# proycon/analiticcl

Hardware: AMD Instinct MI355X
Metric: scored (query,candidate) pairs/sec + queries/sec, 200k-lexicon, len≤16, 1/2/4/8 GPU (higher is better)
Workload: dtype u8

## Files before the change

analiticcl_amd/_lib.py:

```python
from __future__ import annotations

import ctypes as C
import os

HERE = os.path.dirname(os.path.abspath(__file__))
LIB_PATH = os.environ.get("ANX_LIB") or os.path.join(HERE, "libanx.so")

ANX_OK, ANX_EINVAL, ANX_EIO, ANX_ENOTBUILT, ANX_ENODEVICE, ANX_ELIMIT, ANX_EEMPTY = 0, -1, -2, -3, -4, -5, -6
ANX_NO_VIA = 0xFFFFFFFFFFFFFFFF
ABI_VERSION = 3


class AnxError(RuntimeError):
    def __init__(self, code: int, message: str):
        super().__init__(f"anx error {code}: {message}")
        self.code = code


class Weights(C.Structure):
    _fields_ = [("ld", C.c_double), ("lcs", C.c_double), ("prefix", C.c_double), ("suffix", C.c_double),
                ("casew", C.c_double)]


class Threshold(C.Structure):
# ... 92 lines not shown
        "anx_index_read_tag": (C.c_void_p, [cp]),
        "anx_model_num_lexicons": (u64, [vp]),
        "anx_model_lexicon_name": (cp, [vp, u64]),
        "anx_model_to_device": (C.c_int, [vp, C.c_int]),
        "anx_model_to_devices": (C.c_int, [vp, C.POINTER(C.c_int), C.c_int]),
        "anx_model_num_replicas": (C.c_int, [vp]),
        "anx_model_replica_device": (C.c_int, [vp, C.c_int]),
        "anx_debug_set_switch": (C.c_int, [cp, cp]),
        "anx_batch_num_shards": (C.c_int, [vp]),
        "anx_batch_shard_info": (C.c_int, [vp, C.c_int, C.POINTER(C.c_int), C.POINTER(sz), C.POINTER(sz)]),
        "anx_batch_shard_inputs": (C.c_int, [vp, C.c_int, C.POINTER(C.POINTER(C.c_uint32))]),
        "anx_model_has": (C.c_int, [vp, cp]),
        "anx_model_vocab_size": (u64, [vp]),
        "anx_model_vocab_text": (cp, [vp, u64]),
        "anx_model_vocab_frequency": (C.c_uint32, [vp, u64]),
        "anx_model_vocab_lexindex": (C.c_uint32, [vp, u64]),
        "anx_model_num_instances": (u64, [vp]),
        "anx_model_num_classes": (u64, [vp]),
        "anx_model_bucket_size": (u64, [vp, C.c_int]),
        "anx_model_alphabet_size": (C.c_int, [vp]),
        "anx_model_normalize": (C.c_int, [vp, cp, C.c_char_p, C.c_int]),
        "anx_model_anahash": (C.c_int, [vp, cp, C.c_char_p, C.c_int]),
        "anx_find_variants_batch": (C.c_int, [vp, C.POINTER(cp), sz, C.POINTER(Params),
                                              C.POINTER(C.POINTER(Result)), C.POINTER(C.POINTER(sz))]),
        "anx_results_free": (None, [C.POINTER(Result), C.POINTER(sz)]),
        "anx_format_query_output": (C.c_int, [vp, C.POINTER(cp), sz, C.POINTER(Result), C.POINTER(sz), C.c_float, C.c_int,
                                              C.c_int, u64, C.POINTER(C.c_void_p), C.POINTER(sz)]),
        "anx_string_free": (None, [C.c_void_p]),
        "anx_format_search_output": (C.c_int, [vp, C.POINTER(cp), sz, C.POINTER(Match), C.POINTER(sz), C.POINTER(Result),
                                               C.POINTER(MatchTag), C.c_float, C.c_int, C.c_int, u64,
                                               C.POINTER(C.c_void_p), C.POINTER(sz)]),
        "anx_default_search_params": (None, [C.POINTER(SearchParams)]),
        "anx_find_all_matches_batch": (C.c_int, [vp, C.POINTER(cp), sz, C.POINTER(SearchParams),
                                                 C.POINTER(C.POINTER(Match)), C.POINTER(C.POINTER(sz)),
                                                 C.POINTER(C.POINTER(Result)), C.POINTER(sz),
                                                 C.POINTER(C.POINTER(MatchTag))]),
        "anx_matches_free": (None, [C.POINTER(Match), C.POINTER(sz), C.POINTER(Result), C.POINTER(MatchTag)]),
        "anx_model_add_contextrule": (C.c_int, [vp, cp, C.c_float, C.POINTER(cp), sz, C.POINTER(cp), sz]),
        "anx_model_read_contextrules": (C.c_int, [vp, cp]),
        "anx_model_num_tags": (sz, [vp]),
        "anx_model_tag_name": (cp, [vp, sz]),
        "anx_batch_encode": (vp, [vp, C.POINTER(cp), sz, C.POINTER(Params)]),
        "anx_batch_encode_packed": (vp, [vp, C.c_char_p, sz, sz, C.POINTER(Params)]),
        "anx_batch_gather_compact": (C.c_int, [vp, C.c_int, vp, sz, C.POINTER(sz), C.POINTER(sz)]),
        "anx_batch_encode_packed_device": (vp, [vp, vp, sz, sz, C.POINTER(Params)]),
        "anx_batch_encode_packed_device_on": (vp, [vp, vp, sz, sz, C.POINTER(Params), vp]),
        "anx_debug_search_stats": (C.c_int, [C.POINTER(C.c_uint64)]),
        "anx_learn_variants": (C.c_int, [vp, C.POINTER(cp), sz, C.POINTER(Params), C.c_int, C.POINTER(C.c_uint64)]),
        "anx_learn_variants_search": (C.c_int, [vp, C.POINTER(cp), sz, C.POINTER(SearchParams), C.c_int, C.POINTER(C.c_uint64)]),
        "anx_learn_apply_rows": (C.c_int, [vp, C.POINTER(cp), sz, C.POINTER(Result), C.POINTER(sz), C.POINTER(C.c_uint64)]),
        "anx_model_variants": (C.c_int64, [vp, u64, C.POINTER(C.c_uint8), C.POINTER(C.c_uint64), C.POINTER(C.c_double), sz]),
        "anx_model_vocab_type": (C.c_uint32, [vp, u64]),
        "anx_format_variant_list": (C.c_int, [vp, C.c_int, C.POINTER(C.c_void_p)]),
        "anx_debug_learn_stats": (C.c_int, [C.POINTER(C.c_uint64)]),
        "anx_debug_learn_times": (C.c_int, [C.POINTER(C.c_double)]),
        "anx_debug_small_stats": (C.c_int, [C.POINTER(C.c_uint64)]),
        "anx_batch_run": (C.c_int, [vp, vp, vp]),
        "anx_batch_run_async": (C.c_int, [vp, vp, vp]),
        "anx_batch_wait": (C.c_int, [vp, vp]),
        "anx_batch_fetch": (C.c_int, [vp, C.POINTER(C.POINTER(Result)), C.POINTER(C.POINTER(sz))]),
        "anx_batch_fetch_compact": (C.c_int, [vp, C.POINTER(C.c_void_p), C.POINTER(C.POINTER(C.c_uint32))]),
        "anx_compact_free": (None, [C.c_void_p, C.POINTER(C.c_uint32)]),
        "anx_compact_to_results": (None, [C.c_void_p, sz, C.POINTER(Result)]),
        "anx_batch_fetch_pairs": (C.c_int, [vp, C.POINTER(C.POINTER(Pair)), C.POINTER(sz)]),
        "anx_pairs_free": (None, [C.POINTER(Pair)]),
        "anx_batch_pair_counts": (C.c_int, [vp, C.POINTER(C.POINTER(C.c_uint32))]),
        "anx_counts_free": (None, [C.POINTER(C.c_uint32)]),
        "anx_batch_export_topk": (C.c_int, [vp, vp, C.c_uint32, vp]),
        "anx_batch_export_compact": (C.c_int, [vp, vp, sz, vp, C.POINTER(sz)]),
        "anx_batch_get_stats": (C.c_int, [vp, C.POINTER(BatchStats), C.c_size_t]),
        "anx_shutdown": (None, []),
        "anx_pipeline_new": (vp, [vp, C.c_int]),
        "anx_pipeline_submit_packed": (C.c_int, [vp, cp, C.c_size_t, C.c_size_t, C.POINTER(Params)]),
        "anx_pipeline_pending": (C.c_int, [vp]),
        "anx_pipeline_next": (C.c_int, [vp, C.POINTER(vp), C.POINTER(C.POINTER(C.c_uint32)), C.POINTER(C.c_size_t)]),
        "anx_pipeline_free": (None, [vp]),
        "anx_debug_kernel_timer": (None, [C.c_int]),
        "anx_debug_kernel_time": (C.c_int, [cp, C.POINTER(C.c_double), C.POINTER(C.c_uint64)]),
        "anx_debug_length_split": (C.c_int, [vp, C.POINTER(C.c_char_p), C.c_size_t, C.POINTER(Params), C.c_int, vp, vp]),
        "anx_debug_signature": (C.c_int, [vp, cp, C.POINTER(C.c_uint64)]),
        "anx_debug_entries": (C.c_int, [vp, C.POINTER(C.POINTER(C.c_uint32)), C.POINTER(C.c_size_t)]),
        "anx_debug_adjacency": (C.c_int, [vp, C.c_int, C.c_uint64, vp, C.c_size_t, vp, C.POINTER(C.POINTER(C.c_uint32)), vp]),
        "anx_debug_adjacency_device": (C.c_int, [vp, vp, C.c_size_t, vp, C.POINTER(C.POINTER(C.c_uint32))]),
        "anx_debug_band_bound": (C.c_int, [C.c_int, vp, vp, vp, vp, C.c_size_t, C.c_int, C.c_int, vp]),
        "anx_batch_free": (None, [vp]),
        "anx_device_pool_trim": (None, [C.c_int]),
    }
    for name, (res, args) in sig.items():
        fn = getattr(L, name)
        fn.restype = res
        fn.argtypes = args
    _lib = L
    return L


EXPORTED = None


def set_switch(name: str, value) -> None:
    check(lib().anx_debug_set_switch(name.encode(), None if value is None else str(value).encode()))


def kernel_timer(enable: bool) -> None:
    lib().anx_debug_kernel_timer(1 if enable else 0)


def kernel_time(name: str):
    ms, n = C.c_double(0.0), C.c_uint64(0)
    lib().anx_debug_kernel_time(name.encode(), C.byref(ms), C.byref(n))
    return ms.value, n.value


def check(rc: int):
    if rc != 0:
        raise AnxError(rc, lib().anx_last_error().decode("utf-8", "replace"))


def last_error() -> str:
    return lib().anx_last_error().decode("utf-8", "replace")
```

analiticcl_amd/csrc/adjacency.h:

```cpp
#pragma once
#include <cstdint>
#include <cstddef>
#include <vector>

namespace anx {

struct LexiconImage;

constexpr int kAdjRadius = 3;
constexpr int kAdjSections = 2 * kAdjRadius + 1;
constexpr int kAdjMaxClosure = 2;
constexpr uint32_t kAdjRow = 64;

struct AdjHdr {
  uint32_t row0;
  uint32_t cum[kAdjSections];
};
struct AdjSlot {
  uint32_t lo, hi;
  uint32_t hdr1;
  uint32_t rows;
};
struct AdjPlanes { uint32_t p1, p2; };

struct AdjIndex {
  std::vector<AdjSlot> hash;
  uint32_t hash_mask = 0;
  std::vector<AdjHdr> hdr;
  AdjPlanes* planes = nullptr;
  uint32_t* ids = nullptr;
  uint64_t rows = 0;
  uint32_t nsig_lexicon = 0, nsig_closure = 0, nsig_kept = 0;
  uint64_t records = 0;
  uint64_t rows_wanted = 0;
  double len_records[256] = {};
  std::vector<float> class_records;
  std::vector<float> class_nsig;
  double build_ms = 0.0;
  AdjIndex() = default;
  AdjIndex(const AdjIndex&) = delete;
  AdjIndex& operator=(const AdjIndex&) = delete;
  ~AdjIndex();
  uint32_t find(uint32_t lo, uint32_t hi) const;
};

void build_adjacency(const LexiconImage& img, int closure, size_t budget_bytes, unsigned threads, AdjIndex& out);

}
```

analiticcl_amd/csrc/capi.cpp:

```cpp
#include <chrono>
#include <cmath>
#include <cstdlib>
#include <charconv>
#include <cstring>
#include <fstream>
#include <sstream>
#include <string>

#include "engine.h"
#include <algorithm>
#include <atomic>
#include <condition_variable>
#include <deque>
#include <functional>
#include <memory>
#include <mutex>
#include <thread>

#include "host_model.h"

namespace {
struct Worker {
  std::thread th;
  std::mutex mu;
// ... 292 lines not shown
    adj.reset(new anx::AdjIndex());
    anx::build_adjacency(m->host.lex, anx::switches().adj_closure, (size_t)anx::switches().adj_budget_mb << 20, anx::usable_hw_threads(), *adj);
  }
  auto publish = [&](const anx::AdjIndex& a, bool have) {
    LengthCost& lc = m->len_cost;
    std::lock_guard<std::mutex> lk(lc.mu);
    for (uint32_t L = 0; L < LengthCost::LMAX; ++L) lc.records[L] = a.len_records[L];
    lc.class_records = a.class_records;
    lc.class_nsig = a.class_nsig;
    lc.have_records = have;
    lc.init = false;
    if (getenv("ANX_ADJ_TIMING"))
      fprintf(stderr, "[anx adjacency] %s: %u lexicon signatures, %u in the closure, %u lists, %llu records in %llu rows (%.1f MB), %.1f ms\n", on_device ? "device" : "host",
              a.nsig_lexicon, a.nsig_closure, a.nsig_kept, (unsigned long long)a.records, (unsigned long long)a.rows, a.rows * 64.0 * 12.0 / 1e6, a.build_ms);
  };
  if (adj) publish(*adj, !adj->hash.empty());
  for (int i = 0; i < n; ++i) {
    Replica r;
    r.device = devices[i];
    if (on_device && i == 0) stats.reset(new anx::AdjIndex());
    r.dev = anx::lexicon_upload(m->host.lex, et, adj.get(), devices[i], err, on_device ? anx::switches().adj_closure : -1, (size_t)anx::switches().adj_budget_mb << 20,
                                (on_device && i == 0) ? stats.get() : nullptr);
    if (r.dev && on_device && i == 0) publish(*stats, stats->nsig_kept != 0);
    if (r.dev && n > 1 && !(r.stream = anx::stream_create(devices[i], err))) { anx::lexicon_free(r.dev); r.dev = nullptr; }
    if (!r.dev) { drop_replicas(m); return fail(ANX_ENODEVICE, err); }
    if (n > 1) r.worker.reset(new Worker());
    m->replicas.push_back(std::move(r));
  }
  m->dev = m->replicas[0].dev;
  return ANX_OK;
}
int anx_model_to_device(anx_model* m, int device) { return anx_model_to_devices(m, &device, 1); }
int anx_model_num_replicas(const anx_model* m) { return m ? (int)m->replicas.size() : 0; }
int anx_model_replica_device(const anx_model* m, int i) { return (m && i >= 0 && (size_t)i < m->replicas.size()) ? m->replicas[(size_t)i].device : -1; }
int anx_debug_signature(const anx_model* m, const char* utf8, uint64_t* out_sig) {
  if (!m || !utf8 || !out_sig) return fail(ANX_EINVAL, "NULL argument");
  if (!m->host.built) return fail(ANX_ENOTBUILT, "Model has not been built yet!");
  std::vector<uint8_t> norm, cv;
  if (!m->host.encode(utf8, norm, cv)) return fail(ANX_ELIMIT, "more than 255 symbols");
  cv.resize((size_t)m->host.lex.nplanes * 4, 0);
  *out_sig = anx::signature_of(cv.data(), cv.size(), m->host.lex.sym_group);
  return ANX_OK;
}
int anx_debug_entries(const anx_model* m, uint32_t** out_vocab_ids, size_t* n) {
  if (!m || !out_vocab_ids || !n) return fail(ANX_EINVAL, "NULL argument");
  if (!m->host.built) return fail(ANX_ENOTBUILT, "Model has not been built yet!");
  const std::vector<uint32_t>& v = m->host.lex.ent_vocab;
  uint32_t* o = static_cast<uint32_t*>(malloc(std::max<size_t>(v.size(), 1) * sizeof(uint32_t)));
  if (!o) return fail(ANX_ELIMIT, "out of memory");
  if (!v.empty()) memcpy(o, v.data(), v.size() * sizeof(uint32_t));
  *out_vocab_ids = o;
  *n = v.size();
  return ANX_OK;
}
int anx_debug_adjacency(const anx_model* m, int closure, uint64_t budget_bytes, const uint64_t* sigs, size_t n, uint32_t* out_cum, uint32_t** out_ids,
                        uint64_t* out_stats) {
  if (!m || (!sigs && n) || (!out_cum && n) || !out_ids) return fail(ANX_EINVAL, "NULL argument");
  if (!m->host.built) return fail(ANX_ENOTBUILT, "Model has not been built yet!");
  anx::AdjIndex adj;
  anx::build_adjacency(m->host.lex, closure, (size_t)budget_bytes, anx::usable_hw_threads(), adj);
  if (out_stats) { out_stats[0] = adj.nsig_lexicon; out_stats[1] = adj.nsig_closure; out_stats[2] = adj.nsig_kept; out_stats[3] = adj.records; out_stats[4] = adj.rows; out_stats[5] = (uint64_t)adj.build_ms; out_stats[6] = adj.rows_wanted; }
  size_t total = 0;
  std::vector<uint32_t> h1(n);
  for (size_t i = 0; i < n; ++i) {
    h1[i] = adj.find((uint32_t)sigs[i], (uint32_t)(sigs[i] >> 32));
    if (h1[i]) total += (size_t)adj.hdr[h1[i] - 1].cum[anx::kAdjSections - 1] * anx::kAdjRow;
  }
  uint32_t* ids = static_cast<uint32_t*>(malloc(std::max<size_t>(total, 1) * sizeof(uint32_t)));
  if (!ids) return fail(ANX_ELIMIT, "out of memory");
  size_t pos = 0;
  for (size_t i = 0; i < n; ++i) {
    uint32_t* c = out_cum + i * (anx::kAdjSections + 1);
    if (!h1[i]) { for (int s = 0; s <= anx::kAdjSections; ++s) c[s] = 0xFFFFFFFFu; continue; }
    const anx::AdjHdr& h = adj.hdr[h1[i] - 1];
    c[0] = (uint32_t)(pos / anx::kAdjRow);
    for (int s = 0; s < anx::kAdjSections; ++s) c[s + 1] = h.cum[s];
    const size_t cnt = (size_t)h.cum[anx::kAdjSections - 1] * anx::kAdjRow;
    memcpy(ids + pos, adj.ids + (size_t)h.row0 * anx::kAdjRow, cnt * sizeof(uint32_t));
    pos += cnt;
  }
  *out_ids = ids;
  return ANX_OK;
}
int anx_debug_adjacency_device(const anx_model* m, const uint64_t* sigs, size_t n, uint32_t* out_cum, uint32_t** out_ids) {
  if (!m || (!sigs && n) || (!out_cum && n) || !out_ids) return fail(ANX_EINVAL, "NULL argument");
  if (m->replicas.empty()) return fail(ANX_ENODEVICE, "model is not resident on a device");
  std::string err;
  const int rc = anx::adjacency_debug_lists(m->replicas[0].dev, sigs, n, out_cum, out_ids, err);
  return rc ? fail(rc, err) : ANX_OK;
}
int anx_debug_set_switch(const char* name, const char* value) {
  return anx::set_switch(name, value) ? ANX_OK : fail(ANX_EINVAL, "unknown switch");
}
void anx_debug_kernel_timer(int enable) { anx::kernel_timer_enable(enable != 0); }
int anx_debug_small_stats(uint64_t* out) { if (!out) return fail(ANX_EINVAL, "NULL argument"); anx::small_stats(out); return ANX_OK; }
int anx_debug_kernel_time(const char* name, double* total_ms, uint64_t* launches) {
  return anx::kernel_timer_read(name, total_ms, launches) ? ANX_OK : fail(ANX_EINVAL, "no launch of that kernel was timed");
}
int anx_debug_band_bound(int device, const uint8_t* q_rows, const uint8_t* c_rows, const uint8_t* lq, const uint8_t* lc, size_t n, int d, int form,
                         uint8_t* out_reject) {
  if ((!q_rows || !c_rows || !lq || !lc || !out_reject) && n) return fail(ANX_EINVAL, "NULL argument");
  std::string err;
  const int rc = anx::debug_band_bound(device, q_rows, c_rows, lq, lc, n, d, form, out_reject, err);
  return rc ? fail(rc, err) : ANX_OK;
}
int anx_model_build(anx_model* m, int device) {
  if (!m) return fail(ANX_EINVAL, "NULL model");
  std::string err;
  int rc = m->host.build_index(err);
  if (rc) return fail(rc, err);
  drop_replicas(m);
  if (device < 0) return ANX_OK;
  return anx_model_to_device(m, device);
}
int anx_model_save_index(const anx_model* m, const char* path) {
  if (!m || !path) return fail(ANX_EINVAL, "NULL argument");
  std::string err;
  const int rc = m->host.save_index(path, err);
  return rc ? fail(rc, err) : ANX_OK;
}
int anx_model_set_index_tag(anx_model* m, const char* tag) {
  if (!m || !tag) return fail(ANX_EINVAL, "NULL argument");
  m->host.index_tag = tag;
  return ANX_OK;
}
char* anx_index_read_tag(const char* path) {
  if (!path) { fail(ANX_EINVAL, "NULL argument"); return nullptr; }
  std::string tag, err;
  const int rc = anx::index_read_tag(path, &tag, err);
  if (rc) { fail(rc, err); return nullptr; }
  char* out = static_cast<char*>(malloc(tag.size() + 1));
  if (!out) { fail(ANX_EINVAL, "out of memory"); return nullptr; }
  memcpy(out, tag.c_str(), tag.size() + 1);
  return out;
}
int anx_model_load_index(anx_model* m, const char* path, int device) {
  if (!m || !path) return fail(ANX_EINVAL, "NULL argument");
  std::string err;
  const int rc = m->host.load_index(path, err);
  if (rc) return fail(rc, err);
  drop_replicas(m);
  if (device < 0) return ANX_OK;
  return anx_model_to_device(m, device);
}
uint64_t anx_model_num_lexicons(const anx_model* m) { return m ? m->host.lexicons.size() : 0; }
const char* anx_model_lexicon_name(const anx_model* m, uint64_t i) {
  return (m && i < m->host.lexicons.size()) ? m->host.lexicons[i].c_str() : nullptr;
}
int anx_model_has(const anx_model* m, const char* utf8) { return (m && utf8 && m->host.has(utf8)) ? 1 : 0; }
uint64_t anx_model_vocab_size(const anx_model* m) { return m ? m->host.decoder.size() : 0; }
const char* anx_model_vocab_text(const anx_model* m, uint64_t id) {
  return (m && id < m->host.decoder.size()) ? m->host.decoder[id].text.c_str() : nullptr;
}
uint32_t anx_model_vocab_frequency(const anx_model* m, uint64_t id) {
  return (m && id < m->host.decoder.size()) ? m->host.decoder[id].frequency : 0;
}
uint32_t anx_model_vocab_lexindex(const anx_model* m, uint64_t id) {
  return (m && id < m->host.decoder.size()) ? m->host.decoder[id].lexindex : 0;
}
uint64_t anx_model_num_instances(const anx_model* m) { return m ? m->host.lex.nentries : 0; }
uint64_t anx_model_num_classes(const anx_model* m) { return m ? m->host.lex.nclasses : 0; }
uint64_t anx_model_bucket_size(const anx_model* m, int c) {
  if (!m || !m->host.built || c < 0 || c > anx::kMaxSymbols) return 0;
  return m->host.lex.bucket_begin[c + 1] - m->host.lex.bucket_begin[c];
}
int anx_model_alphabet_size(const anx_model* m) { return m ? m->host.alphabet_size() : 0; }
// ... 1404 lines not shown
```

analiticcl_amd/csrc/encode.hip:

```cpp
#include <hip/hip_runtime.h>

#include <cstdio>
#include <cstring>
#include <ctime>
#include <string>
#include <vector>

#include <rocprim/device/device_radix_sort.hpp>
#include <rocprim/device/device_scan.hpp>

#include "engine_internal.h"

namespace anx {

#define HIP_TRY(expr)                                                                          \
  do {                                                                                         \
    hipError_t _e = (expr);                                                                    \
    if (_e != hipSuccess) {                                                                    \
      err = std::string(#expr) + ": " + hipGetErrorString(_e);                                 \
      return ANX_ENODEVICE;                                                                    \
    }                                                                                          \
  } while (0)

#include "kernels_common.hpp"
// ... 295 lines not shown
  const uint32_t meta = g.meta[i], len = meta & 0xFFu;
  const unsigned long long sig = g.sig[i];
  g.q_meta[s] = meta;
  g.q_orig[s] = i;
  g.s_sig[s] = sig;
  static_assert(NBITPLANES == 4, "planes move as one uint4");
  const uint4 planes = reinterpret_cast<const uint4*>(g.bits)[i];
  const uint32_t kind = g.kind[i];
  reinterpret_cast<uint4*>(g.q_bits)[s] = planes;
  g.s_kind[s] = kind;
  if (kind == 0)
    for (int p = 0; p < g.NP; ++p) g.q_cv[(size_t)s * g.NP + p] = g.cv[(size_t)i * g.NP + p];
  const uint32_t* __restrict__ src = reinterpret_cast<const uint32_t*>(g.codes + code_off(g.off[i], i));
  for (uint32_t w = 0; w < g.qw; ++w) {
    const uint32_t left = len > w * 16u ? len - w * 16u : 0u;
    uint32_t v[4];
#pragma unroll
    for (uint32_t x = 0; x < 4u; ++x) {
      const uint32_t word = 4u * x < left ? src[w * 4u + x] : 0u;
      const uint32_t valid = left > 4u * x ? left - 4u * x : 0u;
      const uint32_t mask = valid >= 4u ? 0xFFFFFFFFu : (1u << (8u * valid)) - 1u;
      v[x] = (word & mask) | (0xFEFEFEFEu & ~mask);
    }
    const uint4 row = make_uint4(v[0], v[1], v[2], v[3]);
    g.q_rows[(size_t)s * g.qw + w] = row;
    if (w == 0) {
      uint32_t pw[3] = {0u, 0u, 0u};
      {
        uint32_t p[6] = {0u, 0u, 0u, 0u, 0u, 0u};
#pragma unroll
        for (uint32_t i = 0; i < 16u; ++i) {
          const uint32_t c = ((v[i >> 2] >> (8u * (i & 3u))) & 0xFFu) + 1u;
          const uint32_t on = i < len ? 1u : 0u;
#pragma unroll
          for (uint32_t b = 0; b < 6u; ++b) p[b] |= (((c >> b) & on)) << i;
        }
        pw[0] = p[0] | p[1] << 16; pw[1] = p[2] | p[3] << 16; pw[2] = p[4] | p[5] << 16;
      }
      g.q_rec[2 * (size_t)s] = row;
      g.q_rec[2 * (size_t)s + 1] = make_uint4(meta, pw[0], pw[1], pw[2]);
    }
  }
  uint32_t xc = 0xFFFFFFFFu;
  if (g.want_exact) {
    int lo = (int)g.siglen_begin[len], hi = (int)g.siglen_begin[len + 1] - 1;
    while (lo <= hi) {
      const int mid = (lo + hi) >> 1;
      const uint4 r = g.sigtab[mid];
      const unsigned long long v = (unsigned long long)r.x | (unsigned long long)r.y << 32;
      if (sig < v) hi = mid - 1;
      else if (sig > v) lo = mid + 1;
      else {
        for (uint32_t c = r.z; c < r.z + r.w && xc == 0xFFFFFFFFu; ++c) {
          bool eq = true;
          for (int p = 0; p < g.NP; ++p)
            eq = eq && g.cls_planes[(size_t)p * g.cstride + c] == (kind ? cv_word_of_planes(planes, (uint32_t)p) : g.cv[(size_t)i * g.NP + p]);
          if (eq) xc = c;
        }
        break;
      }
    }
  }
  g.qexact[s] = xc;
}
__global__ __launch_bounds__(256) void k_enc_gather(GatherArgs g) {
  const uint32_t s = blockIdx.x * 256 + threadIdx.x;
  if (s < g.nq) enc_gather_body(g, s);
}

struct TileArgs {
  uint32_t nq, tq;
  const uint32_t *q_meta, *s_kind;
  const unsigned long long* s_sig;
  const uint32_t* siglen_begin;
  uint32_t* head;
  uint32_t* tcount;
  Tile* tiles;
  uint32_t* tkey;
  uint32_t* ctr;
  const uint32_t* ball_tab;
  int probe;
  const uint4* adj_hash;
  uint32_t adj_mask;
};
__device__ inline uint32_t adj_lookup(const uint4* tab, uint32_t mask, uint32_t lo, uint32_t hi, uint32_t* rows) {
  if (!mask) return 0u;
  uint32_t h = sig_hash(lo, hi) & mask;
  for (int p = 0; p < 17; ++p) {
    const uint4 e = tab[h];
    if (!e.z) return 0u;
    if (e.x == lo && e.y == hi) { *rows = e.w; return e.z; }
    h = (h + 1u) & mask;
  }
  return 0u;
}
__device__ inline bool same_segment(const TileArgs& t, uint32_t a, uint32_t b) {
  return (t.s_kind[a] == 0) == (t.s_kind[b] == 0) && (t.q_meta[a] & 0xFFu) == (t.q_meta[b] & 0xFFu) && t.s_sig[a] == t.s_sig[b];
}
__device__ inline void tile_window(const TileArgs& t, uint32_t s, uint32_t& s0, uint32_t& s1, uint32_t& step, uint32_t& nparts,
                                   uint32_t& ball0, uint32_t& balln) {
  const uint32_t meta = t.q_meta[s], lq = meta & 0xFFu, k = (meta >> 8) & 0xFFu;
  const int lo = max(1, (int)lq - (int)k), hi = min(kMaxSymbols, (int)lq + (int)k);
  s0 = t.siglen_begin[lo] & ~63u;
  s1 = (t.siglen_begin[hi + 1] + 63u) & ~63u;
  ball0 = balln = 0;
  if (t.probe && k <= 12u && tile_probes(t.ball_tab[13 + k], s1 - s0, t.s_sig[s])) { ball0 = t.ball_tab[k]; balln = t.ball_tab[13 + k]; }
  const uint32_t nsplit = (t.s_kind[s] == 0 && !balln) ? 8u : 1u;
  step = (((s1 - s0) + nsplit - 1u) / nsplit + 63u) & ~63u;
  nparts = 0;
  for (uint32_t part = 0; part < nsplit; ++part) {
    const uint32_t a0 = s0 + part * step, a1 = min(s1, a0 + step);
    if (a0 >= a1 && part) break;
    ++nparts;
  }
}
__global__ __launch_bounds__(256) void k_tile_heads(TileArgs t) {
  const uint32_t s = blockIdx.x * 256 + threadIdx.x;
  if (s >= t.nq) return;
  t.head[s] = (s > 0 && !same_segment(t, s, s - 1)) ? s : 0u;
}
__global__ __launch_bounds__(256) void k_tile_count(TileArgs t) {
  const uint32_t s = blockIdx.x * 256 + threadIdx.x;
  if (s > t.nq) return;
  uint32_t c = 0;
  if (s < t.nq && (s - t.head[s]) % t.tq == 0) {
    uint32_t s0, s1, step, nparts, ball0, balln;
    tile_window(t, s, s0, s1, step, nparts, ball0, balln);
    c = nparts;
  }
  t.tcount[s] = c;
}
__global__ __launch_bounds__(256) void k_tile_emit(TileArgs t) {
  const uint32_t s = blockIdx.x * 256 + threadIdx.x;
  if (s >= t.nq || (s - t.head[s]) % t.tq != 0) return;
  const uint32_t hs = t.head[s];
  uint32_t lo = s + 1u, hi = min(s + t.tq, t.nq);
  while (lo < hi) {
    const uint32_t mid = (lo + hi) >> 1;
    if (t.head[mid] != hs) hi = mid; else lo = mid + 1u;
  }
  const uint32_t tn = lo - s;
  uint32_t ke[3];
#pragma unroll
  for (uint32_t v = 1; v <= 3u; ++v) {
    uint32_t a = s, b = s + tn;
    while (a < b) {
      const uint32_t mid = (a + b) >> 1;
      if (t.s_kind[mid] > v) b = mid; else a = mid + 1u;
    }
    ke[v - 1] = a - s;
  }
  const bool sad = t.s_kind[s] == 0;
  const uint32_t meta = t.q_meta[s], lq = meta & 0xFFu, k = (meta >> 8) & 0xFFu, d = (meta >> 16) & 0xFFu;
  uint32_t s0, s1, step, nparts, ball0, balln;
  tile_window(t, s, s0, s1, step, nparts, ball0, balln);
  const unsigned long long sig = t.s_sig[s];
  const uint32_t base = t.tcount[s];
  uint32_t adj_rows = 0;
  const uint32_t adj = (!sad && k <= (uint32_t)kAdjRadius) ? adj_lookup(t.adj_hash, t.adj_mask, (uint32_t)sig, (uint32_t)(sig >> 32), &adj_rows) : 0u;
  for (uint32_t part = 0; part < nparts; ++part) {
    const uint32_t a0 = s0 + part * step, a1 = min(s1, a0 + step);
    Tile tl;
    tl.q0 = s; tl.nq = tn; tl.s0 = a0; tl.s1 = a1; tl.k = k; tl.lq = lq; tl.sig_lo = (uint32_t)sig; tl.sig_hi = (uint32_t)(sig >> 32);
    tl.kind = sad ? 0u : 1u; tl.d = d; tl.kend = sad ? 0u : (ke[0] | ke[1] << 8 | ke[2] << 16);
    tl.ball0 = ball0; tl.balln = balln; tl.adj = adj; tl.flags = (s == hs && part == 0u) ? 1u : 0u;
    t.tiles[base + part] = tl;
    const unsigned long long cost = adj ? (unsigned long long)adj_rows * (8u + tn) + 16u : (unsigned long long)tn * (a1 - a0 + 64u);
    t.tkey[base + part] = (sad ? 0x80000000u : adj ? 0u : 0x40000000u) | (0x3FFFFFFFu - (uint32_t)(cost < 0x3FFFFFFFull ? cost : 0x3FFFFFFFull));
  }
  if (sad) atomicAdd(&t.ctr[3], nparts);
}

__global__ __launch_bounds__(256) void k_tile_adj_count(const Tile* tiles, uint32_t n, uint32_t* ctr) {
  const uint32_t i = blockIdx.x * 256 + threadIdx.x;
  if (i < n && tiles[i].adj && (i + 1 == n || !tiles[i + 1].adj)) ctr[5] = i + 1u;
}

__global__ __launch_bounds__(256) void k_small_tiles(GatherArgs g, TileArgs t, SmallZero z, uint32_t slots, const uint32_t* __restrict__ adj_hdr) {
  const uint32_t s = blockIdx.x * 256 + threadIdx.x, nthreads = gridDim.x * 256u;
#pragma unroll
  for (int a = 0; a < 8; ++a)
    for (uint32_t i = s; i < z.n[a]; i += nthreads) z.p[a][i] = 0u;
  if (s >= t.nq) return;
  enc_gather_body(g, s);
  const uint32_t meta = t.q_meta[s], lq = meta & 0xFFu, k = (meta >> 8) & 0xFFu, d = (meta >> 16) & 0xFFu;
  Tile nul{};
  nul.kind = 1u;
  uint32_t nparts = 0;
  if (meta) {
    const uint32_t kind = t.s_kind[s];
    const bool sad = kind == 0;
    uint32_t s0, s1, step, ball0, balln;
    tile_window(t, s, s0, s1, step, nparts, ball0, balln);
    const unsigned long long sig = t.s_sig[s];
    uint32_t adj_rows = 0;
    const uint32_t adj = (!sad && k <= (uint32_t)kAdjRadius) ? adj_lookup(t.adj_hash, t.adj_mask, (uint32_t)sig, (uint32_t)(sig >> 32), &adj_rows) : 0u;
    uint32_t rbeg = 0, rend = 0;
    if (adj) {
      const uint32_t* hp = adj_hdr + (size_t)(adj - 1u) * 8u;
      rbeg = k >= 3u ? 0u : k == 2u ? hp[1] : k == 1u ? hp[2] : hp[3];
      rend = k >= 3u ? hp[7] : k == 2u ? hp[6] : k == 1u ? hp[5] : hp[4];
      const uint32_t rows = rend > rbeg ? rend - rbeg : 0u;
      nparts = min(slots, max(1u, rows / 8u));
      step = ((rows + nparts - 1u) / nparts + 3u) & ~3u;
    }
    for (uint32_t part = 0; part < nparts; ++part) {
      const uint32_t a0 = s0 + part * step, a1 = min(s1, a0 + step);
      Tile tl;
      tl.q0 = s; tl.nq = 1u; tl.s0 = a0; tl.s1 = a1; tl.k = k; tl.lq = lq; tl.sig_lo = (uint32_t)sig; tl.sig_hi = (uint32_t)(sig >> 32);
      tl.kind = sad ? 0u : 1u; tl.d = d;
      tl.kend = sad ? 0u : ((kind <= 1u ? 1u : 0u) | (kind <= 2u ? 1u : 0u) << 8 | (kind <= 3u ? 1u : 0u) << 16);
      tl.ball0 = ball0; tl.balln = balln; tl.adj = adj; tl.flags = part == 0u ? 1u : 0u;
      if (adj) {
        tl.s0 = min(rend, rbeg + part * step);
        tl.s1 = min(rend, tl.s0 + step);
        tl.flags |= 2u;
        if (tl.s0 >= tl.s1 && part) tl.nq = 0u;
      }
      t.tiles[(size_t)part * t.nq + s] = tl;
    }
  }
  (void)nul;
  for (uint32_t part = nparts; part < slots; ++part) t.tiles[(size_t)part * t.nq + s].nq = 0u;
}

int small_encode_launch(const HostModel& m, const DeviceLexicon* dl, const SmallEnc& e, const uint8_t* blob, const uint32_t* off, uint32_t n, uint32_t qw,
                        const anx_params& p, const SmallZero& z, uint32_t slots, bool stage_lds, const uint32_t* host_off, hipStream_t st, std::string& err) {
  const int NP = dl->nplanes;
  EncArgs ea;
  ea.blob = blob; ea.off = off; ea.n = n; ea.al = dl->alpha; ea.A = m.alphabet.size(); ea.NP = NP;
  ea.bits_ok = (dl->nsym <= 32 && !switches().scan_sad) ? 1 : 0;
  ea.ngroups = 1;
  for (uint8_t g : m.lex.sym_group) ea.ngroups = std::max(ea.ngroups, (int)g + 1);
  ea.kth = p.max_anagram_distance; ea.dth = p.max_edit_distance;
  ea.codes = e.codes; ea.meta = e.meta; ea.bits = e.bits; ea.sig = e.sig; ea.kind = e.kind; ea.cv = e.cv; ea.key = e.key; ea.blk = e.blk;
  ea.dbg = 0;
  ea.zero_cv = 1;
  for (uint32_t bk = 0; bk <= 16u; ++bk) ea.stage_off[bk] = host_off ? host_off[std::min<uint32_t>(bk * 256u, n)] : 0u;
  const dim3 gn((n + 255) / 256);
  if (stage_lds && host_off && n <= 4096u) hipLaunchKernelGGL(k_enc_strings<true>, gn, dim3(256), 0, st, ea);
  else hipLaunchKernelGGL(k_enc_strings<false>, gn, dim3(256), 0, st, ea);
  GatherArgs ga;
  ga.nq = n; ga.qw = qw; ga.NP = NP; ga.want_exact = 0;
  ga.perm = e.perm; ga.off = off; ga.codes = e.codes; ga.meta = e.meta; ga.bits = e.bits; ga.kind = e.kind; ga.cv = e.cv; ga.sig = e.sig;
  ga.q_rec = e.q_rec; ga.q_rows = e.q_rows; ga.q_bits = e.q_bits; ga.q_cv = e.q_cv; ga.q_meta = e.q_meta; ga.q_orig = e.q_orig;
  ga.qexact = e.qexact; ga.s_kind = e.s_kind; ga.s_sig = e.s_sig;
  ga.sigtab = dl->sig; ga.siglen_begin = dl->alpha.siglen_begin; ga.cls_planes = dl->cls_planes; ga.cstride = dl->cstride;
  TileArgs ta;
  ta.tq = 1; ta.nq = n; ta.q_meta = e.q_meta; ta.s_kind = e.s_kind; ta.s_sig = e.s_sig; ta.siglen_begin = dl->alpha.siglen_begin; ta.ctr = nullptr;
  ta.ball_tab = dl->ball_tab; ta.probe = probe_enabled() ? 1 : 0;
  ta.adj_hash = dl->adj_hash; ta.adj_mask = switches().scan_adj ? dl->adj_mask : 0u;
  ta.head = nullptr; ta.tcount = nullptr; ta.tiles = e.tiles; ta.tkey = nullptr;
  hipLaunchKernelGGL(k_small_tiles, gn, dim3(256), 0, st, ga, ta, z, slots, dl->adj_hdr);
  HIP_TRY(hipGetLastError());
  return ANX_OK;
}
int small_iota(uint32_t* perm, uint32_t n, hipStream_t st) {
  hipLaunchKernelGGL(k_iota, dim3((n + 255) / 256), dim3(256), 0, st, perm, n);
  return hipGetLastError() == hipSuccess ? ANX_OK : ANX_ENODEVICE;
}

namespace {
struct Scratch {
  std::vector<void*> blocks;
  int device;
  hipStream_t st;
  explicit Scratch(int dev) : device(dev), st(encoder_stream_acquire(dev)) {}
  template <typename T>
  int get(T** p, size_t count, std::string& err) {
    void* q = nullptr;
    HIP_TRY(pool_malloc(&q, std::max<size_t>(count * sizeof(T), 16)));
    blocks.push_back(q);
    *p = static_cast<T*>(q);
    return ANX_OK;
  }
  ~Scratch() { (void)hipStreamSynchronize(st); for (void* q : blocks) pool_free(q); encoder_stream_release(device, st); }
};
template <typename K>
int sort_pairs(const K* kin, K* kout, const uint32_t* vin, uint32_t* vout, size_t n, unsigned b0, unsigned b1, Scratch& sc, hipStream_t st,
               std::string& err) {
  size_t bytes = 0;
  HIP_TRY(rocprim::radix_sort_pairs(nullptr, bytes, kin, kout, vin, vout, n, b0, b1, st));
  char* tmp = nullptr;
  int rc = sc.get(&tmp, bytes + 16, err);
  if (rc) return rc;
  HIP_TRY(rocprim::radix_sort_pairs(tmp, bytes, kin, kout, vin, vout, n, b0, b1, st));
  return ANX_OK;
}
template <typename T>
int balloc(T** dst, size_t count, std::string& err) {
  HIP_TRY(pool_malloc(reinterpret_cast<void**>(dst), std::max<size_t>(count * sizeof(T), 16)));
  return ANX_OK;
}
}

int batch_encode_device(const HostModel& m, const DeviceLexicon* dl, Batch* b, const char* blob, size_t blob_bytes, const uint32_t* off,
                        size_t n, const anx_params& p, std::string& err, bool blob_on_device, bool after_stream, void* src_stream) {
  const bool timing = switches().encode_timing != 0;
  double t_prev = 0.0;
  auto tnow = []() { timespec ts; clock_gettime(CLOCK_MONOTONIC, &ts); return ts.tv_sec + 1e-9 * ts.tv_nsec; };
  if (timing) t_prev = tnow();
  Scratch sc(dl->device);
  hipStream_t st = sc.st;
  auto lap = [&](const char* what) { if (timing) { (void)hipStreamSynchronize(st); const double t = tnow(); fprintf(stderr, "[anx encode/device] %-24s %8.2f ms\n", what, (t - t_prev) * 1e3); t_prev = t; } };
  const uint32_t n32 = (uint32_t)n;
  const size_t blob_len = !n ? 0 : off ? off[n] : blob_bytes;
  const int NP = dl->nplanes;
  int rc;
  if (blob_len + 4 * (size_t)n + 16 >= ((size_t)1 << 32)) { err = "inputs exceed 4 GB per batch (bytes + 4 per string): split the batch"; return ANX_ELIMIT; }
  if (n == 0) {
    b->nq = 0; b->dmax = 0; b->qw = 1; b->ntiles = 0; b->n_sad_tiles = 0; b->n_adj_tiles = 0;
    if ((rc = balloc(&b->q_rec, 0, err)) || (rc = balloc(&b->qexact, 0, err)) || (rc = balloc(&b->q_cv, 0, err)) || (rc = balloc(&b->q_bits, 0, err)) ||
        (rc = balloc(&b->q_rows, 0, err)) || (rc = balloc(&b->q_meta, 0, err)) || (rc = balloc(&b->q_orig, 0, err)) || (rc = balloc(&b->d_tiles, 0, err)))
      return rc;
    return ANX_OK;
  }
  uint8_t *d_blob = nullptr, *d_codes = nullptr;
  uint32_t *d_off = nullptr, *d_meta = nullptr, *d_bits = nullptr, *d_kind = nullptr, *d_cv = nullptr, *d_ctr = nullptr, *d_blk = nullptr;
  unsigned long long* d_key = nullptr;
  unsigned long long* d_sig = nullptr;
  if (b->keep_text) {
    if ((rc = balloc(&b->d_text, blob_len + 16, err)) || (rc = balloc(&b->d_textoff, n + 1, err))) return rc;
    d_blob = b->d_text;
    d_off = b->d_textoff;
    b->text_bytes = blob_len;
  } else if ((rc = sc.get(&d_blob, blob_len + 16, err)) || (rc = sc.get(&d_off, n + 1, err))) return rc;
  if ((rc = sc.get(&d_codes, blob_len + 4 * (size_t)n + 16, err)) ||
      (rc = sc.get(&d_meta, n, err)) || (rc = sc.get(&d_bits, n * NBITPLANES, err)) || (rc = sc.get(&d_kind, n, err)) ||
      (rc = sc.get(&d_cv, n * (size_t)NP, err)) || (rc = sc.get(&d_key, n, err)) || (rc = sc.get(&d_sig, n, err)) || (rc = sc.get(&d_ctr, 8, err)) ||
      (rc = sc.get(&d_blk, 3 * ((n + 255) / 256), err)))
    return rc;
  if (after_stream) {
    hipEvent_t ev = nullptr;
    HIP_TRY(hipEventCreateWithFlags(&ev, hipEventDisableTiming));
    hipError_t e1 = hipEventRecord(ev, reinterpret_cast<hipStream_t>(src_stream));
    if (e1 == hipSuccess) e1 = hipStreamWaitEvent(st, ev, 0);
// ... 2 lines not shown
  }
  HIP_TRY(hipMemcpyAsync(d_blob, blob, blob_len, blob_on_device ? hipMemcpyDeviceToDevice : hipMemcpyHostToDevice, st));
  const int bits_ok = (dl->nsym <= 32 && !switches().scan_sad) ? 1 : 0;
  if (!bits_ok) HIP_TRY(hipMemsetAsync(d_cv, 0, n * (size_t)NP * 4, st));
  HIP_TRY(hipMemsetAsync(d_ctr, 0, 8 * sizeof(uint32_t), st));
  if (off) {
    HIP_TRY(hipMemcpyAsync(d_off, off, (n + 1) * sizeof(uint32_t), hipMemcpyHostToDevice, st));
  } else {
    const uint32_t nblk = (uint32_t)((blob_len + NUL_BLK - 1) / NUL_BLK);
    uint32_t* d_cnt = nullptr;
    if ((rc = sc.get(&d_cnt, nblk, err))) return rc;
    hipLaunchKernelGGL(k_nul_count, dim3(nblk), dim3(256), 0, st, d_blob, (uint32_t)blob_len, d_cnt, d_ctr + 4);
    size_t bytes = 0;
    HIP_TRY(rocprim::exclusive_scan(nullptr, bytes, d_cnt, d_cnt, 0u, (size_t)nblk, rocprim::plus<uint32_t>(), st));
    char* tmp = nullptr;
    if ((rc = sc.get(&tmp, bytes + 16, err))) return rc;
    HIP_TRY(rocprim::exclusive_scan(tmp, bytes, d_cnt, d_cnt, 0u, (size_t)nblk, rocprim::plus<uint32_t>(), st));
    hipLaunchKernelGGL(k_nul_emit, dim3(nblk), dim3(256), 0, st, d_blob, (uint32_t)blob_len, d_cnt, n32, d_off);
    uint32_t have = 0;
    HIP_TRY(hipMemcpyAsync(&have, d_ctr + 4, sizeof have, hipMemcpyDeviceToHost, st));
    HIP_TRY(hipStreamSynchronize(st));
    if (have < n) { err = "packed inputs hold fewer strings than announced"; return ANX_EINVAL; }
  }
  EncArgs ea;
  ea.blob = d_blob; ea.off = d_off; ea.n = n32; ea.al = dl->alpha; ea.A = m.alphabet.size(); ea.NP = NP;
  ea.bits_ok = bits_ok;
  ea.ngroups = 1;
  for (uint8_t g : m.lex.sym_group) ea.ngroups = std::max(ea.ngroups, (int)g + 1);
  ea.kth = p.max_anagram_distance; ea.dth = p.max_edit_distance;
  ea.codes = d_codes; ea.meta = d_meta; ea.bits = d_bits; ea.sig = d_sig; ea.kind = d_kind; ea.cv = d_cv; ea.key = d_key; ea.blk = d_blk;
  ea.dbg = 0;
  ea.zero_cv = 0;
#ifdef ANX_DEBUG_SWITCHES
  { const char* e = getenv("ANX_ENC_DBG"); ea.dbg = e ? atoi(e) : 0; }
#endif
  const dim3 gn((n32 + 255) / 256);
  lap("alloc + H2D");
  hipLaunchKernelGGL(k_enc_strings<false>, gn, dim3(256), 0, st, ea);
  hipLaunchKernelGGL(k_enc_totals, dim3(1), dim3(256), 0, st, d_blk, gn.x, d_ctr);
  lap("k_enc_strings");
  uint32_t *perm_a = nullptr, *perm_b = nullptr;
  unsigned long long* k64_b = nullptr;
  if ((rc = sc.get(&perm_a, n, err)) || (rc = sc.get(&perm_b, n, err)) || (rc = sc.get(&k64_b, n, err))) return rc;
  hipLaunchKernelGGL(k_iota, gn, dim3(256), 0, st, perm_a, n32);
  if ((rc = sort_pairs(d_key, k64_b, perm_a, perm_b, n, 0, 13 + 5 * ea.ngroups, sc, st, err))) return rc;
  const uint32_t* perm = perm_b;
  uint32_t h_ctr[8];
  HIP_TRY(hipMemcpyAsync(h_ctr, d_ctr, sizeof h_ctr, hipMemcpyDeviceToHost, st));
  HIP_TRY(hipStreamSynchronize(st));
  lap("sort");
  const uint32_t nq = h_ctr[2];
  b->nq = nq;
  b->dmax = h_ctr[1];
  b->qw = (std::max<uint32_t>(h_ctr[0], 1u) + 15u) / 16u;
  uint32_t* s_kind = nullptr;
  unsigned long long* s_sig = nullptr;
  if ((rc = sc.get(&s_kind, nq, err)) || (rc = sc.get(&s_sig, nq, err))) return rc;
  if ((rc = balloc(&b->q_rec, 2 * (size_t)nq, err)) || (rc = balloc(&b->qexact, nq, err)) || (rc = balloc(&b->q_cv, (size_t)nq * NP, err)) ||
      (rc = balloc(&b->q_bits, (size_t)nq * NBITPLANES, err)) || (rc = balloc(&b->q_rows, (size_t)nq * b->qw, err)) ||
      (rc = balloc(&b->q_meta, nq, err)) || (rc = balloc(&b->q_orig, nq, err)))
    return rc;
  b->ntiles = 0;
  b->n_sad_tiles = 0;
  b->n_adj_tiles = 0;
  if (nq == 0) {
    if ((rc = balloc(&b->d_tiles, 0, err))) return rc;
    HIP_TRY(hipStreamSynchronize(st));
    return ANX_OK;
  }
  GatherArgs ga;
  ga.nq = nq; ga.qw = b->qw; ga.NP = NP; ga.want_exact = p.stop_at_exact_match ? 1 : 0;
  ga.perm = perm; ga.off = d_off; ga.codes = d_codes; ga.meta = d_meta; ga.bits = d_bits; ga.kind = d_kind; ga.cv = d_cv; ga.sig = d_sig;
  ga.q_rec = b->q_rec; ga.q_rows = b->q_rows; ga.q_bits = b->q_bits; ga.q_cv = b->q_cv; ga.q_meta = b->q_meta; ga.q_orig = b->q_orig;
  ga.qexact = b->qexact; ga.s_kind = s_kind; ga.s_sig = s_sig;
  ga.sigtab = dl->sig; ga.siglen_begin = dl->alpha.siglen_begin; ga.cls_planes = dl->cls_planes; ga.cstride = dl->cstride;
  const dim3 gq((nq + 255) / 256);
  hipLaunchKernelGGL(k_enc_gather, gq, dim3(256), 0, st, ga);
  lap("k_enc_gather");
  TileArgs ta;
  ta.tq = switches().scan_tq ? (uint32_t)switches().scan_tq : default_scan_tq(ea.ngroups);
  ta.nq = nq; ta.q_meta = b->q_meta; ta.s_kind = s_kind; ta.s_sig = s_sig; ta.siglen_begin = dl->alpha.siglen_begin; ta.ctr = d_ctr;
  ta.ball_tab = dl->ball_tab; ta.probe = probe_enabled() ? 1 : 0;
  ta.adj_hash = dl->adj_hash; ta.adj_mask = switches().scan_adj ? dl->adj_mask : 0u;
  uint32_t *d_head = nullptr, *d_tcount = nullptr;
  if ((rc = sc.get(&d_head, nq, err)) || (rc = sc.get(&d_tcount, (size_t)nq + 1, err))) return rc;
  ta.head = d_head; ta.tcount = d_tcount; ta.tiles = nullptr; ta.tkey = nullptr;
  hipLaunchKernelGGL(k_tile_heads, gq, dim3(256), 0, st, ta);
  {
    size_t bytes = 0;
    HIP_TRY(rocprim::inclusive_scan(nullptr, bytes, d_head, d_head, (size_t)nq, rocprim::maximum<uint32_t>(), st));
    char* tmp = nullptr;
    if ((rc = sc.get(&tmp, bytes + 16, err))) return rc;
    HIP_TRY(rocprim::inclusive_scan(tmp, bytes, d_head, d_head, (size_t)nq, rocprim::maximum<uint32_t>(), st));
  }
  hipLaunchKernelGGL(k_tile_count, dim3((nq + 1 + 255) / 256), dim3(256), 0, st, ta);
  {
    size_t bytes = 0;
    HIP_TRY(rocprim::exclusive_scan(nullptr, bytes, d_tcount, d_tcount, 0u, (size_t)nq + 1, rocprim::plus<uint32_t>(), st));
    char* tmp = nullptr;
    if ((rc = sc.get(&tmp, bytes + 16, err))) return rc;
    HIP_TRY(rocprim::exclusive_scan(tmp, bytes, d_tcount, d_tcount, 0u, (size_t)nq + 1, rocprim::plus<uint32_t>(), st));
  }
  uint32_t ntiles = 0;
  HIP_TRY(hipMemcpyAsync(&ntiles, d_tcount + nq, sizeof(uint32_t), hipMemcpyDeviceToHost, st));
  HIP_TRY(hipStreamSynchronize(st));
  Tile *t_unsorted = nullptr;
  uint32_t *tkey_a = nullptr, *tkey_b = nullptr, *tperm_a = nullptr, *tperm_b = nullptr;
  if ((rc = sc.get(&t_unsorted, ntiles, err)) || (rc = sc.get(&tkey_a, ntiles, err)) || (rc = sc.get(&tkey_b, ntiles, err)) ||
      (rc = sc.get(&tperm_a, ntiles, err)) || (rc = sc.get(&tperm_b, ntiles, err)) || (rc = balloc(&b->d_tiles, ntiles, err)))
    return rc;
  ta.tiles = t_unsorted; ta.tkey = tkey_a;
  hipLaunchKernelGGL(k_tile_emit, gq, dim3(256), 0, st, ta);
  if (ntiles) {
    const dim3 gt((ntiles + 255) / 256);
    hipLaunchKernelGGL(k_iota, gt, dim3(256), 0, st, tperm_a, ntiles);
    if ((rc = sort_pairs(tkey_a, tkey_b, tperm_a, tperm_b, ntiles, 0, 32, sc, st, err))) return rc;
    hipLaunchKernelGGL(k_gather<Tile>, gt, dim3(256), 0, st, t_unsorted, tperm_b, b->d_tiles, ntiles);
    hipLaunchKernelGGL(k_tile_adj_count, gt, dim3(256), 0, st, b->d_tiles, ntiles, d_ctr);
  }
  HIP_TRY(hipMemcpyAsync(h_ctr, d_ctr, sizeof h_ctr, hipMemcpyDeviceToHost, st));
  HIP_TRY(hipStreamSynchronize(st));
  HIP_TRY(hipGetLastError());
  b->ntiles = ntiles;
  b->n_sad_tiles = h_ctr[3];
  b->n_adj_tiles = h_ctr[5];
  lap("tiles");
  return ANX_OK;
}

}
```

analiticcl_amd/csrc/engine.hip:

```cpp
#include <hip/hip_runtime.h>

#include <algorithm>
#include <atomic>
#include <functional>
#include <chrono>
#include <cmath>
#include <cstdio>
#include <cstdlib>
#include <cstring>
#include <map>
#include <memory>
#include <mutex>
#include <unordered_map>
#include <numeric>
#include <thread>
#include <type_traits>

#include "engine_internal.h"

namespace anx {

#define HIP_TRY(expr)                                                                          \
  do {                                                                                         \
    hipError_t _e = (expr);                                                                    \
// ... 720 lines not shown
      for (unsigned t = 0; t < nthreads; ++t) th.emplace_back(sort_buckets, t);
    for (auto& x : th) x.join();
  }
  lap("signature sort");
  auto fill_range = [&](size_t lo, size_t hi) {
    for (size_t s = lo; s < hi; ++s) {
      if (s + 8 < hi) {
        const size_t ip = b->order[s + 8];
        __builtin_prefetch(&enc[ip]);
        __builtin_prefetch(&cv_all[ip * cvbytes]);
      }
      if (s + 4 < hi) { const Enc& ep = enc[b->order[s + 4]]; __builtin_prefetch(&arena[ep.thread][ep.off]); }
      const size_t i = b->order[s];
      const Enc& e = enc[i];
      const uint8_t* cv = &cv_all[i * cvbytes];
      memcpy(&h_cv[s * (size_t)NP], cv, cvbytes);
      for (uint32_t tp = 0; tp < (uint32_t)NBITPLANES; ++tp) h_bits[s * NBITPLANES + tp] = 0;
      for (size_t sym = 0; sym < cvbytes && sym < 32; ++sym) {
        const uint32_t c = cv[sym];
        for (uint32_t tp = 0; tp < c && tp < (uint32_t)NBITPLANES; ++tp) h_bits[s * NBITPLANES + tp] |= 1u << sym;
      }
      uint8_t* row = &h_rows[s * (size_t)b->qw * 16];
      memset(row, 0xFE, (size_t)b->qw * 16);
      memcpy(row, &arena[e.thread][e.off], e.meta & 0xFF);
      memcpy(&h_qrec[2 * s], row, 16);
      {
        uint32_t pw[3];
        symbol_planes16(reinterpret_cast<const uint8_t*>(row), e.meta & 0xFFu, pw);
        h_qrec[2 * s + 1] = make_uint4(e.meta, pw[0], pw[1], pw[2]);
      }
      h_meta[s] = e.meta;
      h_orig[s] = (uint32_t)i;
      h_kind[s] = e.kind;
      h_sig[s] = e.sig;
    }
  };
  {
    std::vector<std::thread> th;
    for (unsigned t = 0; t < nthreads; ++t) {
      const size_t lo = nq * t / nthreads, hi = nq * (t + 1) / nthreads;
      if (nthreads == 1) fill_range(lo, hi);
      else th.emplace_back(fill_range, lo, hi);
    }
    for (auto& x : th) x.join();
  }
  lap("fill device images");
  for (size_t i = 0; i < nq;) {
    size_t j = i;
    const bool sad = h_kind[i] == 0;
    while (j < nq && (h_kind[j] == 0) == sad && (h_meta[j] & 0xFF) == (h_meta[i] & 0xFF) && h_sig[j] == h_sig[i]) ++j;
    const uint32_t lq = h_meta[i] & 0xFF, k = (h_meta[i] >> 8) & 0xFF;
    const int lo = std::max<int>(1, (int)lq - (int)k), hi = std::min<int>(kMaxSymbols, (int)lq + (int)k);
    const uint32_t s0 = m.lex.siglen_begin[lo] & ~63u, s1 = (m.lex.siglen_begin[hi + 1] + 63u) & ~63u;
    uint32_t ngroups_ = 1;
    for (uint8_t g_ : m.lex.sym_group) ngroups_ = std::max<uint32_t>(ngroups_, (uint32_t)g_ + 1u);
    const uint32_t tq = switches().scan_tq ? (uint32_t)switches().scan_tq : default_scan_tq((int)ngroups_);
    uint32_t ball0 = 0, balln = 0;
    if (probe_enabled() && k <= 12 && tile_probes(dl->ball_n[k], s1 - s0, h_sig[i])) { ball0 = dl->ball_off[k]; balln = dl->ball_n[k]; }
    const uint32_t nsplit = (sad && !balln) ? 8u : 1u;
    const uint32_t step = (((s1 - s0) + nsplit - 1) / nsplit + 63u) & ~63u;
    uint32_t adj = 0;
    if (!sad && k <= (uint32_t)kAdjRadius && switches().scan_adj && dl->adj_mask && dl->adj_hash_host.empty()) {
      const int rca = adjacency_host_copies(dl, err);
      if (rca) return rca;
    }
    if (!sad && k <= (uint32_t)kAdjRadius && switches().scan_adj && !dl->adj_hash_host.empty()) {
      uint32_t h = sig_hash((uint32_t)h_sig[i], (uint32_t)(h_sig[i] >> 32)) & dl->adj_mask;
      for (int pr = 0; pr < 17; ++pr) {
        const AdjSlot& e = dl->adj_hash_host[h];
        if (!e.hdr1) break;
        if (e.lo == (uint32_t)h_sig[i] && e.hi == (uint32_t)(h_sig[i] >> 32)) { adj = e.hdr1; break; }
        h = (h + 1u) & dl->adj_mask;
      }
    }
    for (size_t s = i; s < j; s += tq) {
      const uint32_t tn = (uint32_t)std::min<size_t>(tq, j - s);
      uint32_t ke[3] = {0, 0, 0};
      for (uint32_t x = 0; x < tn; ++x)
        for (uint32_t kd = h_kind[s + x]; kd >= 1 && kd <= 3; ++kd) ke[kd - 1]++;
      const uint32_t kend = sad ? 0u : (ke[0] | ke[1] << 8 | ke[2] << 16);
      for (uint32_t part = 0; part < nsplit; ++part) {
        const uint32_t a0 = s0 + part * step, a1 = std::min(s1, a0 + step);
        if (a0 >= a1 && part) break;
        b->tiles.push_back(Tile{(uint32_t)s, tn, a0, a1, k, lq, (uint32_t)h_sig[i], (uint32_t)(h_sig[i] >> 32), sad ? 0u : 1u,
                                (h_meta[i] >> 16) & 0xFFu, kend, ball0, balln, adj, (s == i && part == 0u) ? 1u : 0u});
      }
    }
    i = j;
  }
  auto tile_cost = [&](const Tile& x) {
    return x.adj ? (uint64_t)dl->adj_hdr_host[x.adj - 1].cum[kAdjSections - 1] * (8u + x.nq) + 16u : (uint64_t)x.nq * (x.s1 - x.s0 + 64);
  };
  std::stable_sort(b->tiles.begin(), b->tiles.end(), [&](const Tile& x, const Tile& y) {
    if ((x.kind == 0) != (y.kind == 0)) return y.kind == 0;
    if ((x.adj == 0) != (y.adj == 0)) return y.adj == 0;
    return tile_cost(x) > tile_cost(y);
  });
  b->n_adj_tiles = 0;
  for (const Tile& t : b->tiles) { b->n_sad_tiles += t.kind == 0; b->n_adj_tiles += t.adj != 0; }
  lap("tiles + LPT order");
  std::vector<uint32_t> h_xcls(nq, 0xFFFFFFFFu);
  if (p.stop_at_exact_match) {
    auto lookup_range = [&](size_t lo, size_t hi) {
      std::string key(cvbytes, '\0');
      for (size_t s = lo; s < hi; ++s) {
        memcpy(&key[0], &cv_all[(size_t)b->order[s] * cvbytes], cvbytes);
        auto it = m.class_of_cv.find(key);
        if (it != m.class_of_cv.end()) h_xcls[s] = it->second;
      }
    };
    std::vector<std::thread> th;
    for (unsigned t = 0; t < nthreads; ++t) {
      const size_t lo = nq * t / nthreads, hi = nq * (t + 1) / nthreads;
      if (nthreads == 1) lookup_range(lo, hi);
      else th.emplace_back(lookup_range, lo, hi);
    }
    for (auto& x : th) x.join();
  }
  int rc;
  if ((rc = upload(&b->q_rec, h_qrec.data(), h_qrec.size(), err, nullptr)) ||
      (rc = upload(&b->qexact, h_xcls.data(), nq, err, nullptr)) ||
      (rc = upload(&b->q_cv, h_cv.data(), h_cv.size(), err, nullptr)) ||
      (rc = upload(&b->q_bits, h_bits.data(), h_bits.size(), err, nullptr)) ||
      (rc = upload(reinterpret_cast<uint8_t**>(&b->q_rows), h_rows.data(), h_rows.size(), err, nullptr)) ||
      (rc = upload(&b->q_meta, h_meta.data(), nq, err, nullptr)) || (rc = upload(&b->q_orig, h_orig.data(), nq, err, nullptr)) ||
      (rc = upload(&b->d_tiles, b->tiles.data(), b->tiles.size(), err, nullptr)))
    return rc;
  b->ntiles = (uint32_t)b->tiles.size();
  std::vector<Tile>().swap(b->tiles);
  lap("uploads");
  return ANX_OK;
}

static int shell_acquire(Batch* b, std::string& err) {
  DevPool& pl = pool_of(b->device);
  BatchShell sh;
  bool have = false;
  {
    std::lock_guard<std::mutex> g(pl.mu);
    if (!pl.shells.empty()) { sh = pl.shells.back(); pl.shells.pop_back(); have = true; }
  }
  if (!have) {
    for (auto& e : sh.ev) HIP_TRY(hipEventCreate(&e));
    HIP_TRY(hipEventCreate(&sh.ev_fs0));
    HIP_TRY(hipEventCreate(&sh.ev_fs1));
    HIP_TRY(hipEventCreate(&sh.ev_scan0));
    HIP_TRY(hipEventCreate(&sh.ev_done));
    HIP_TRY(hipEventCreateWithFlags(&sh.ev_in, hipEventDisableTiming));
    HIP_TRY(hipHostMalloc(reinterpret_cast<void**>(&sh.h_read), HR_COLD_OFF + sizeof(FsCold), hipHostMallocDefault));
  }
  for (int i = 0; i < 6; ++i) b->ev[i] = sh.ev[i];
  b->ev_fs0 = sh.ev_fs0; b->ev_fs1 = sh.ev_fs1; b->ev_scan0 = sh.ev_scan0; b->ev_done = sh.ev_done; b->ev_in = sh.ev_in; b->h_read = sh.h_read;
  return ANX_OK;
}
static void shell_release(Batch* b) {
  if (!b->ev_done) return;
  BatchShell sh;
  for (int i = 0; i < 6; ++i) { sh.ev[i] = b->ev[i]; b->ev[i] = nullptr; }
  sh.ev_fs0 = b->ev_fs0; sh.ev_fs1 = b->ev_fs1; sh.ev_scan0 = b->ev_scan0; sh.ev_done = b->ev_done; sh.ev_in = b->ev_in; sh.h_read = b->h_read;
  b->ev_fs0 = b->ev_fs1 = b->ev_scan0 = b->ev_done = b->ev_in = nullptr; b->h_read = nullptr;
  DevPool& pl = pool_of(b->device);
  std::lock_guard<std::mutex> g(pl.mu);
  pl.shells.push_back(sh);
}
static void shells_destroy(int device) {
  DevPool& pl = pool_of(device);
  std::vector<BatchShell> drop;
  { std::lock_guard<std::mutex> g(pl.mu); drop.swap(pl.shells); }
// ... 260 lines not shown
         h.score_threshold == b->params.score_threshold && h.stop == (b->params.stop_at_exact_match ? 1 : 0) && h.seg == seg_wanted(b);
}
static void hints_apply(const DeviceLexicon* dl, Batch* b) {
  if (b->runs_finished || b->hinted || b->prev_maxfill || !switches().hints || switches().cap_div != 1 || b->nq < 4096) return;
  RunHints& h = dl->hints;
  std::lock_guard<std::mutex> g(h.mu);
  if (!hints_match(h, b)) return;
  const double nq = (double)b->nq, m = 1.25;
  const double worst_fill = (nq * 140.0 + (double)b->ntiles * SCAN_CHUNK) / SCAN_REGIONS + 4096.0;
  const double fill = h.maxfill * nq * m + 8192.0;
  if (fill >= worst_fill) return;
  b->prev_maxfill = (uint32_t)fill;
  b->prev_surv_fill = (uint32_t)(h.surv_fill * nq * m + 1024.0);
  b->prev_list_fill = h.list_fill > 0 ? (uint32_t)(h.list_fill * nq * m + 1024.0) : 0u;
  b->hint_rows = (size_t)std::min(nq * 16.0 + 1024.0, h.total_surv * nq * m + 4096.0);
  b->hinted = true;
}
static void hints_record(const DeviceLexicon* dl, const Batch* b, uint32_t maxfill, uint32_t surv_fill, uint32_t list_fill, uint32_t total_surv) {
  if (b->nq < 4096 || !switches().hints) return;
  RunHints& h = dl->hints;
  std::lock_guard<std::mutex> g(h.mu);
  const double nq = (double)b->nq, decay = hints_match(h, b) ? 0.9 : 0.0;
  h.maxfill = std::max(maxfill / nq, h.maxfill * decay);
  h.surv_fill = std::max(surv_fill / nq, h.surv_fill * decay);
  h.list_fill = std::max(list_fill / nq, h.list_fill * decay);
  h.total_surv = std::max(total_surv / nq, h.total_surv * decay);
  h.kth = b->params.max_anagram_distance; h.dth = b->params.max_edit_distance; h.score_threshold = b->params.score_threshold;
  h.stop = b->params.stop_at_exact_match ? 1 : 0;
  h.seg = seg_wanted(b);
  h.nq = nq;
  h.valid = true;
}

static int batch_launch(const HostModel& m, const DeviceLexicon* dl, Batch* b, void* stream, std::string& err) {
  if (!dl) { err = "model is not resident on a device"; return ANX_ENODEVICE; }
  if (b->nq >= (1u << 27) || dl->nentries >= (1u << 26)) { err = "more than 2^27 queries per batch or 2^26 lexicon entries (32-bit record offsets, packed pair records)"; return ANX_ELIMIT; }
  HIP_TRY(hipSetDevice(dl->device));
  hipStream_t st = reinterpret_cast<hipStream_t>(stream);
  const uint32_t nq = (uint32_t)b->nq;
  if (b->launched) {
    HIP_TRY(hipEventSynchronize(b->ev_done));
    b->launched = false;
  }
  b->last_stream = stream;
  b->ran = false;
  b->ran_keep_all = b->keep_all_pairs;
  b->n_pairs = b->n_results = b->n_surv = 0;
  b->n_raw = 0;
  if (nq == 0) { b->ran = true; return ANX_OK; }
  const int stop = b->params.stop_at_exact_match ? 1 : 0;
  int rc;
  hints_apply(dl, b);
  if (b->raw_cap == 0 && b->hinted && (rc = ensure_raw(b, (size_t)b->prev_maxfill + (b->prev_maxfill >> 3) + 4096, err))) return rc;
  if (b->raw_cap == 0 && (rc = ensure_raw(b, (nq * (size_t)140 + (size_t)b->ntiles * SCAN_CHUNK) / SCAN_REGIONS / cap_div() + 4096, err)))
    return rc;
  const uint32_t region_cap = 1u << b->region_shift;
  const uint32_t fill_cap = b->prev_maxfill ? (uint32_t)std::min<size_t>(region_cap, (size_t)b->prev_maxfill + (b->prev_maxfill >> 3) + FS_BLK) : region_cap;
  b->fill_cap_launched = fill_cap;
  HIP_TRY(hipEventRecord(b->ev[0], st));
  HIP_TRY(hipMemsetAsync(b->counters, 0, CTR_N * sizeof(uint32_t), st));
  HIP_TRY(hipMemsetAsync(b->rctr, 0, SCAN_REGIONS * RC_STRIDE * sizeof(uint32_t), st));
  if (b->ntiles == 0) { HIP_TRY(hipEventRecord(b->ev_scan0, st)); HIP_TRY(hipEventRecord(b->ev[5], st)); }
  if (b->ntiles) {
    ScanArgs A;
    A.tiles = b->d_tiles; A.ntiles = b->ntiles; A.q_bits = b->q_bits; A.q_cv = b->q_cv;
    A.cls_bits = dl->cls_bits; A.cls_planes = dl->cls_planes; A.scan_rec = dl->scan_rec; A.scan_rec34 = dl->scan_rec34; A.pad_rec = dl->nentries; A.cstride = dl->cstride; A.pad_class = dl->nclasses;
    A.cls_len = dl->cls_len; A.cls_off = dl->cls_off; A.sig = dl->sig; A.sig_e = dl->sig_e; A.sig_cbeg = dl->sig_cbeg; A.sighash = dl->sighash; A.sighash_e = dl->sighash_e; A.hash_mask = dl->hash_mask; A.ball = dl->ball;
    A.adj_hdr = dl->adj_hdr; A.adj_planes = dl->adj_planes; A.adj_ids = dl->adj_ids;
    A.chunk = SCAN_CHUNK;
    A.chunk_fused = switches().scan_chunk_fused ? (uint32_t)switches().scan_chunk_fused : SCAN_CHUNK_FUSED;
#ifdef ANX_DEBUG_SWITCHES
    { const char* e = getenv("ANX_SCAN_CHUNK"); const int v = e ? atoi(e) : 0; if (v >= 32 && v <= 1024) A.chunk = (uint32_t)v; }
#endif
    A.raw = b->raw; A.region_cap = region_cap; A.rctr = b->rctr; A.qexact = b->qexact; A.want_exact = stop;
    A.drop_len = (!stop && !b->keep_all_pairs) ? 1 : 0;
    A.q_rec = b->q_rec; A.e_rec = dl->e_rec;
    A.fuse = (switches().fuse_prefilter && switches().prefilter && A.drop_len) ? 1 : 0;
    A.qpairs = nullptr;
    if (b->count_pairs) {
      if (!b->qpairs && (rc = dalloc(&b->qpairs, nq, err))) return rc;
      HIP_TRY(hipMemsetAsync(b->qpairs, 0, nq * sizeof(uint32_t), st));
      A.qpairs = b->qpairs;
    }
    A.dbg = 0;
#ifdef ANX_DEBUG_SWITCHES
    { const char* e = getenv("ANX_SCAN_DBG"); A.dbg = e ? atoi(e) : 0; }
#endif
    const uint32_t nsad = b->n_sad_tiles, nbits = A.ntiles - nsad, nadj = std::min(b->n_adj_tiles, nbits);
    switch (dl->nplanes) {
      case 8: launch_scan<8>(A, nadj, nbits, nsad, st, b->ev_scan0, b->ev[5]); break;
      case 16: launch_scan<16>(A, nadj, nbits, nsad, st, b->ev_scan0, b->ev[5]); break;
      case 24: launch_scan<24>(A, nadj, nbits, nsad, st, b->ev_scan0, b->ev[5]); break;
      case 32: launch_scan<32>(A, nadj, nbits, nsad, st, b->ev_scan0, b->ev[5]); break;
      default: launch_scan<42>(A, nadj, nbits, nsad, st, b->ev_scan0, b->ev[5]); break;
    }
  }
  HIP_TRY(hipMemcpyAsync(b->h_read + HR_RCTR, b->rctr, SCAN_REGIONS * RC_STRIDE * sizeof(uint32_t), hipMemcpyDeviceToHost, st));
  HIP_TRY(hipEventRecord(b->ev[1], st));
  b->n_raw = (uint32_t)(SCAN_REGIONS << b->region_shift);
  HIP_TRY(hipMemsetAsync(b->qsurv, 0, nq * sizeof(uint32_t), st));
  HIP_TRY(hipMemsetAsync(b->qmaxfreq, 0, nq * sizeof(uint32_t), st));
  if (dl->any_variants) HIP_TRY(hipMemsetAsync(b->qexpand, 0, nq * sizeof(uint32_t), st));
  ScoreArgs sa;
  sa.dbg = 0;
#ifdef ANX_DEBUG_SWITCHES
  { const char* e = getenv("ANX_SCORE_DBG"); sa.dbg = e ? atoi(e) : 0; }
#endif
  sa.quot = dl->quot;
  sa.store_pairs = b->keep_all_pairs ? 1 : 0;
  if (sa.store_pairs && (rc = ensure_pair_outputs(b, err))) return rc;
  sa.w_ld = m.weights.ld; sa.w_lcs = m.weights.lcs; sa.w_prefix = m.weights.prefix; sa.w_suffix = m.weights.suffix;
  sa.w_case = m.weights.casew;
  sa.w_sum = m.weights.ld + m.weights.lcs + m.weights.prefix + m.weights.suffix + m.weights.casew;
  sa.score_threshold = b->params.score_threshold;
  sa.have_freq = m.have_freq ? 1 : 0;
  sa.any_variants = dl->any_variants;
  sa.lqp = b->qw * 16;
  sa.lcp = (dl->max_len + 15) / 16 * 16;
  const uint32_t d = b->dmax;
  uint32_t stride = sa.lqp + sa.lcp + (d + 2) * (2 * d + 3);
  stride = (stride + 3) / 4;
  if ((stride & 1) == 0) stride++;
  sa.stride = stride * 4;
  sa.qw = b->qw;
  uint32_t threads = 256;
  while (threads > 64 && (size_t)threads * sa.stride > 64 * 1024) threads >>= 1;
  if ((size_t)threads * sa.stride > 64 * 1024) { err = "per-lane scoring state exceeds the LDS budget"; return ANX_ELIMIT; }
  SurvOut so{nullptr, b->sctr, 0, nullptr, 0};
  const bool have_long_q = b->qw > 1;
  {
    const int enable_filter = switches().prefilter, enable_fast = switches().score_fast;
    const int fastD = (enable_fast && d >= 1 && d <= 3) ? (int)d : 0;
    {
      const size_t need = b->prev_surv_fill ? (size_t)b->prev_surv_fill + (b->prev_surv_fill >> 3) + 256 : (size_t)fill_cap / 2 / cap_div() + 256;
      if (need > b->surv_region_cap) {
        if (b->surv) pool_free(b->surv);
        b->surv = nullptr;
        b->surv_region_cap = 0;
        if ((rc = dalloc(&b->surv, need * SCAN_REGIONS, err))) return rc;
        b->surv_region_cap = need;
      }
    }
    so.list = b->surv;
    so.region_cap = (uint32_t)b->surv_region_cap;
    so.seg_cap = seg_capacity(dl, b);
    so.seg = so.seg_cap ? b->sseg : nullptr;
    const bool need_lists = !fastD || have_long_q || dl->max_len > 16;
    if (need_lists) {
      const size_t need = b->prev_list_fill ? (size_t)b->prev_list_fill + (b->prev_list_fill >> 3) + 256 : (fastD ? (size_t)fill_cap / 2 : (size_t)fill_cap) / cap_div() + 256;
      if (need > b->list_cap) {
        for (void* p : {(void*)b->list8, (void*)b->listg, (void*)b->listw})
          if (p) pool_free(p);
        b->list8 = b->listg = b->listw = nullptr;
        b->list_cap = 0;
        if ((rc = dalloc(&b->list8, need * SCAN_REGIONS, err)) || (rc = dalloc(&b->listg, need * SCAN_REGIONS, err)) ||
            (rc = dalloc(&b->listw, need * SCAN_REGIONS, err))) return rc;
        b->list_cap = need;
      }
    }
    HIP_TRY(hipMemsetAsync(b->sctr, 0, SCAN_REGIONS * RC_STRIDE * sizeof(uint32_t), st));
    HIP_TRY(hipMemsetAsync(b->lctr, 0, 3 * SCAN_REGIONS * RC_STRIDE * sizeof(uint32_t), st));
    const SlotList l8{b->list8, b->lctr, (uint32_t)b->list_cap}, lg{b->listg, b->lctr + SCAN_REGIONS * RC_STRIDE, (uint32_t)b->list_cap},
                   lw{b->listw, b->lctr + 2 * SCAN_REGIONS * RC_STRIDE, (uint32_t)b->list_cap};
    const PairArgs pa{b->raw, b->q_meta, b->q_rows, b->q_rec, dl->e_rec, dl->ent_meta, dl->ent_rowoff, dl->rows, dl->ent_freq, dl->ent_var_off,
                      b->p_score, b->p_meta, b->qmaxfreq, b->qsurv, b->qexpand, dl->e_planes};
    FilterArgs fa;
// ... 566 lines not shown
```

analiticcl_amd/csrc/host_model.cpp:

```cpp
#include "host_model.h"
#include "adjacency.h"

#include <sched.h>

#include <thread>

#include <algorithm>
#include <cmath>
#include <cstdio>
#include <cstring>
#include <fstream>
#include <numeric>
#include <sstream>

#include "unicode_tables.inc"

namespace anx {

static std::vector<uint32_t> make_primes() {
  std::vector<uint32_t> p;
  for (uint32_t n = 2; p.size() < 168; ++n) {
    bool prime = true;
    for (uint32_t d : p) {
      if (d * d > n) break;
// ... 415 lines not shown
    }
    VocabEntry& v = decoder[l.var];
    v.variants.push_back(VariantRef{true, l.ref, l.score});
    v.has_variants = true;
  }
  built = false;
  return f.var_of.size();
}

int HostModel::read_variants(const char* path, const anx_vocab_params& p0, bool transparent, std::string& err) {
  std::string data;
  if (!read_file(path, data)) { err = std::string("cannot read ") + path; return ANX_EIO; }
  std::vector<std::string> lines;
  split_lines(data, lines);
  const uint8_t lexidx = (uint8_t)lexicons.size();
  anx_vocab_params p = p0, tp = p0;
  if (transparent) tp.vocab_type |= ANX_VOCAB_TRANSPARENT;
  int has_freq = -1;
  auto parse_u32 = [](const std::string& f, uint32_t& out) {
    if (f.empty() || f[0] == '-' ) return false;
    char* endp = nullptr;
    unsigned long long v = strtoull(f.c_str() + (f[0] == '+' ? 1 : 0), &endp, 10);
    if (*endp || v > 0xFFFFFFFFull) return false;
    out = (uint32_t)v;
    return true;
  };
  std::vector<std::string> fields;
  size_t linenr = 0;
  for (const std::string& line : lines) {
    ++linenr;
    if (line.empty()) continue;
    fields.clear();
    size_t pos = 0;
    for (;;) {
      size_t e = line.find('\t', pos);
      fields.emplace_back(line, pos, e == std::string::npos ? std::string::npos : e - pos);
      if (e == std::string::npos) break;
      pos = e + 1;
    }
    bool havef = false;
    uint32_t freq = 0;
    if (has_freq < 0) {
      if (fields.size() >= 2 && (fields.size() - 2) % 3 == 0) {
        if (parse_u32(fields[1], freq)) { has_freq = 1; havef = true; }
      } else has_freq = 0;
    } else if (has_freq == 1) {
      if (fields.size() < 2 || !parse_u32(fields[1], freq)) {
        err = "Frequency must be an integer (line " + std::to_string(linenr) + ", column 2)";
        return ANX_EINVAL;
      }
      havef = true;
    }
    const uint64_t ref_id = add_to_vocabulary(fields[0].c_str(), havef, freq, p, lexidx);
    const size_t step = has_freq == 1 ? 3 : 2;
    for (size_t i = has_freq == 1 ? 2 : 1; i + step - 1 < fields.size(); i += step) {
      char* endp = nullptr;
      const double score = strtod(fields[i + 1].c_str(), &endp);
      if (fields[i + 1].empty() || *endp) { err = "Variant scores must be a floating point value (line " + std::to_string(linenr) + ")"; return ANX_EINVAL; }
      uint32_t vf = 0;
      if (has_freq == 1 && !parse_u32(fields[i + 2], vf)) { err = "Variant frequency must be an integer (line " + std::to_string(linenr) + ")"; return ANX_EINVAL; }
      add_variant(ref_id, fields[i].c_str(), score, has_freq == 1, vf, transparent ? tp : p, lexidx);
    }
  }
  lexicons.push_back(path);
  return ANX_OK;
}

static int pick_planes(int nsym) {
  const int need = (nsym + 3) / 4;
  for (int v : {8, 16, 24, 32, 42})
    if (need <= v) return v;
  return -1;
}

namespace {
struct SwitchDef { const char* name; void (*set)(Switches&, const char*); };
int flag01(const char* v, int dflt) { return !v ? dflt : (v[0] == '0' ? 0 : 1); }
const SwitchDef kSwitches[] = {
    {"ANX_ENCODE", [](Switches& s, const char* v) { s.encode_host = v && strcmp(v, "host") == 0; }},
    {"ANX_SCAN", [](Switches& s, const char* v) { s.scan_sad = v && strcmp(v, "sad") == 0; }},
    {"ANX_SCAN_WALK", [](Switches& s, const char* v) { s.scan_walk_flat = v && strcmp(v, "flat") == 0; }},
    {"ANX_SCAN_TQ", [](Switches& s, const char* v) { const int x = v ? atoi(v) : 0; s.scan_tq = x >= 1 && x <= 64 ? x : 0; }},
    {"ANX_SCAN_ADJ", [](Switches& s, const char* v) { s.scan_adj = flag01(v, 1); }},
    {"ANX_ADJ_BUILD", [](Switches& s, const char* v) { s.adj_build_host = v && strcmp(v, "host") == 0; }},
    {"ANX_ADJ_CLOSURE", [](Switches& s, const char* v) { const int x = v ? atoi(v) : 2; s.adj_closure = x >= 0 && x <= kAdjMaxClosure ? x : kAdjMaxClosure; }},
    {"ANX_SCAN_CHUNK_FUSED", [](Switches& s, const char* v) { const int x = v ? atoi(v) : 0; s.scan_chunk_fused = x >= 32 && x <= 1024 ? x : 0; }},
    {"ANX_ADJ_FAIL", [](Switches& s, const char* v) { s.adj_fail = flag01(v, 0); }},
    {"ANX_SMALL", [](Switches& s, const char* v) { s.small_path = flag01(v, 1); }},
    {"ANX_SURV_SEG", [](Switches& s, const char* v) { const int x = v ? atoi(v) : 32; s.surv_seg = x >= 0 && x <= 256 ? x : 32; }},
    {"ANX_ENC_PRIORITY", [](Switches& s, const char* v) { s.enc_priority = flag01(v, 1); }},
    {"ANX_HINTS", [](Switches& s, const char* v) { s.hints = flag01(v, 1); }},
    {"ANX_ADJ_MB", [](Switches& s, const char* v) { const long x = v ? atol(v) : 0; s.adj_budget_mb = x > 0 ? x : 16384; }},
    {"ANX_SIG_GROUPS", [](Switches& s, const char* v) { const int x = v ? atoi(v) : 0; s.sig_groups = x >= 1 && x <= 8 ? x : 0; }},
    {"ANX_PREFILTER", [](Switches& s, const char* v) { s.prefilter = flag01(v, 1); }},
    {"ANX_SCORE_FAST", [](Switches& s, const char* v) { s.score_fast = flag01(v, 1); }},
    {"ANX_FS_SPLIT", [](Switches& s, const char* v) { s.fs_split = flag01(v, 1); }},
    {"ANX_FS_PLANES", [](Switches& s, const char* v) { s.fs_planes = flag01(v, 1); }},
    {"ANX_FS_B7", [](Switches& s, const char* v) { s.fs_b7 = flag01(v, 1); }},
    {"ANX_SCAN_FUSE", [](Switches& s, const char* v) { s.fuse_prefilter = flag01(v, 1); }},
    {"ANX_CAP_DIV", [](Switches& s, const char* v) { const long x = v ? atol(v) : 0; s.cap_div = x > 1 ? x : 1; }},
    {"ANX_MAX_BATCH", [](Switches& s, const char* v) { const long x = v ? atol(v) : 0; s.max_batch = x > 0 ? x : (4l << 20); }},
    {"ANX_RUN_OVERLAP", [](Switches& s, const char* v) { s.run_overlap = (v && atoi(v) == 0 && v[0] == '0') ? 0 : 1; }},
    {"ANX_SHARD_POLICY", [](Switches& s, const char* v) { s.shard_by_length = (v && strcmp(v, "range") == 0) ? 0 : 1; }},
    {"ANX_SHARD_MIN", [](Switches& s, const char* v) { const long x = v ? atol(v) : 0; s.shard_min = x > 0 ? x : 8192; }},
    {"ANX_CONFUSABLES", [](Switches& s, const char* v) { s.confusables_host = v && strcmp(v, "host") == 0; }},
    {"ANX_LATTICE", [](Switches& s, const char* v) { s.lattice_host = v && strcmp(v, "host") == 0; }},
    {"ANX_SEARCH_ONEPASS", [](Switches& s, const char* v) { s.search_onepass = flag01(v, 1); }},
    {"ANX_ENCODE_TIMING", [](Switches& s, const char* v) { s.encode_timing = v != nullptr && v[0] != 0 && v[0] != '0'; }},
    {"ANX_SEARCH_TIMING", [](Switches& s, const char* v) { s.search_timing = v != nullptr && v[0] != 0 && v[0] != '0'; }},
    {"ANX_SEARCH_PARTS", [](Switches& s, const char* v) { const int x = v ? atoi(v) : 0; s.search_parts = x >= 1 && x <= 8 ? x : 4; }},
    {"ANX_SEARCH_PART_BYTES", [](Switches& s, const char* v) { const long x = v ? atol(v) : 0; s.search_part_bytes = x > 0 ? x : (4l << 20); }},
    {"ANX_SEARCH_PRIO", [](Switches& s, const char* v) { s.search_prio = flag01(v, 1); }},
    {"ANX_SEARCH_EARLY_OUTPUT", [](Switches& s, const char* v) { s.search_early_output = flag01(v, 1); }},
    {"ANX_SEARCH_FIRST_PCT", [](Switches& s, const char* v) { const int x = v ? atoi(v) : 0; s.search_first_pct = x >= 10 && x <= 100 ? x : 50; }},
    {"ANX_SEARCH_PARTS_MIN", [](Switches& s, const char* v) { const long x = v ? atol(v) : 0; s.search_parts_min = x > 0 ? x : (2l << 20); }},
    {"ANX_LEARN_FOLD", [](Switches& s, const char* v) { s.learn_fold_host = v && strcmp(v, "host") == 0; }},
};
}
Switches& switches() {
  static Switches sw = []() {
    Switches s;
    for (const SwitchDef& d : kSwitches)
      if (const char* v = getenv(d.name)) d.set(s, v);
    return s;
  }();
  return sw;
}
bool set_switch(const char* name, const char* value) {
  if (!name) return false;
  for (const SwitchDef& d : kSwitches)
    if (strcmp(d.name, name) == 0) { d.set(switches(), value); return true; }
  return false;
}

unsigned usable_hw_threads() {
  static const unsigned cached = []() {
    unsigned n = std::max(1u, std::thread::hardware_concurrency());
    cpu_set_t set;
    if (sched_getaffinity(0, sizeof set, &set) == 0) n = std::min<unsigned>(n, (unsigned)std::max(1, CPU_COUNT(&set)));
    if (FILE* f = fopen("/sys/fs/cgroup/cpu.max", "r")) {
      char q[32];
      long period = 0;
      if (fscanf(f, "%31s %ld", q, &period) == 2 && strcmp(q, "max") != 0 && period > 0) {
        const long quota = atol(q);
        if (quota > 0) n = std::min<unsigned>(n, (unsigned)std::max(1L, (quota + period - 1) / period));
      }
      fclose(f);
    } else {
      long quota = -1, period = 0;
      if (FILE* g = fopen("/sys/fs/cgroup/cpu/cpu.cfs_quota_us", "r")) { if (fscanf(g, "%ld", &quota) != 1) quota = -1; fclose(g); }
      if (FILE* g = fopen("/sys/fs/cgroup/cpu/cpu.cfs_period_us", "r")) { if (fscanf(g, "%ld", &period) != 1) period = 0; fclose(g); }
      if (quota > 0 && period > 0) n = std::min<unsigned>(n, (unsigned)std::max(1L, (quota + period - 1) / period));
    }
    return n;
  }();
  return cached;
}

uint64_t signature_of(const uint8_t* cv, size_t n, const std::vector<uint8_t>& sym_group) {
  uint8_t g[8] = {};
  for (size_t sl = 0; sl < n; ++sl) g[sym_group[sl]] = (uint8_t)(g[sym_group[sl]] + cv[sl]);
  uint64_t s = 0;
  for (int i = 0; i < 8; ++i) s |= (uint64_t)g[i] << (8 * i);
  return s;
}

// ... 228 lines not shown
```

analiticcl_amd/csrc/host_model.h:

```cpp
#pragma once
#include <cstdint>
#include <atomic>
#include <memory>
#include <mutex>
#include <string>
#include <unordered_map>
#include <vector>

#include "../../include/anx.h"
#include "confusables_core.hpp"

namespace anx {

constexpr int kMaxSymbols = 255;
constexpr int kMaxAlphabet = 166;
constexpr int kMaxAnagramDistance = 12;
constexpr int kMaxEditDistance = 12;

struct AlphabetMember {
  std::string bytes;
  int nchars;
};

struct Alphabet {
  std::vector<std::vector<AlphabetMember>> classes;
  int size() const { return (int)classes.size(); }
  struct Cand { int16_t cls; const AlphabetMember* m; };
  std::vector<Cand> by_first[256];
  int16_t fast[256];
  void index();
  bool scan(const char* text, size_t nbytes, std::vector<int16_t>& out) const;
  int scan_into(const char* text, size_t nbytes, int16_t* out, int cap) const;
};

bool parse_alphabet(const std::string& tsv, Alphabet& out, std::string& err);
struct EncodeTables {
  int16_t fast[256];
  uint32_t coff[257];
  std::vector<uint32_t> cand;
  std::vector<uint8_t> bytes;
  std::vector<uint32_t> lower;
};
void build_encode_tables(const Alphabet& a, EncodeTables& out);
bool first_char_is_lowercase(const char* utf8);
bool is_alphabetic_cp(uint32_t cp);
const uint32_t (*alphabetic_ranges(uint32_t* n))[2];
uint32_t utf8_decode_at(const char* s, size_t avail, int* len);
std::string trim_whitespace(const std::string& s);
unsigned usable_hw_threads();

struct Switches {
  int encode_host = 0;
  int scan_sad = 0;
  int scan_walk_flat = 0;
  int scan_tq = 0;
  int scan_adj = 1;
  int adj_build_host = 0;
  int adj_closure = 2;
  long adj_budget_mb = 16384;
  int sig_groups = 0;
  int prefilter = 1;
  int score_fast = 1;
  int fs_planes = 1;
  int fs_split = 1;
  int fs_b7 = 1;
  int fuse_prefilter = 1;
  long cap_div = 1;
  long max_batch = 4l << 20;
  int run_overlap = 1;
  int shard_by_length = 1;
  long shard_min = 8192;
  int confusables_host = 0;
  int lattice_host = 0;
  int search_onepass = 1;
  int scan_chunk_fused = 0;
  int adj_fail = 0;
  int small_path = 1;
  int enc_priority = 1;
  int hints = 1;
  int encode_timing = 0;
  int search_timing = 0;
  int search_parts = 4;
  long search_parts_min = 2l << 20;
  long search_part_bytes = 4l << 20;
  int search_prio = 1;
  int search_early_output = 1;
  int search_first_pct = 50;
  int surv_seg = 32;
  int learn_fold_host = 0;
};
Switches& switches();
bool set_switch(const char* name, const char* value);

struct VariantRef {
  bool variant_of;
  uint64_t id;
  double score;
};

struct VocabEntry {
  std::string text;
  std::vector<uint8_t> norm;
  uint32_t frequency;
  uint32_t lexindex;
  uint8_t tokencount;
  uint8_t vocabtype;
  bool has_variants = false;
  std::vector<VariantRef> variants;
};

struct BigVal {
  std::vector<uint32_t> w;
  void set_one() { w.assign(1, 1u); }
  void mul_small(uint32_t m);
  int cmp(const BigVal& o) const;
  std::string to_decimal() const;
};

struct LexiconImage {
  int nsym = 0;
  int nplanes = 0;
  uint32_t nclasses = 0, nentries = 0;
  std::vector<uint32_t> cls_planes;
  uint32_t cstride = 0;
  std::vector<uint32_t> cls_bits;
  std::vector<uint8_t> cls_len;
  std::vector<uint32_t> cls_off;
  uint32_t bucket_begin[kMaxSymbols + 2];
  std::vector<uint32_t> ent_vocab;
  std::vector<uint32_t> ent_freq;
  std::vector<uint32_t> ent_meta;
  std::vector<uint32_t> ent_var_off;
  std::vector<uint32_t> var_target;
  std::vector<uint32_t> var_target_freq;
  std::vector<double> var_score;
  bool any_variants = false;
  std::vector<uint32_t> ent_rowoff;
  std::vector<uint32_t> ent_order;
  std::vector<uint8_t> rows;
// ... 132 lines not shown
```

analiticcl_amd/csrc/kernels_common.hpp:

```cpp
#pragma once

struct Tile {
  uint32_t q0, nq;
  uint32_t s0, s1;
  uint32_t k;
  uint32_t lq;
  uint32_t sig_lo, sig_hi;
  uint32_t kind;
  uint32_t d;
  uint32_t kend;
  uint32_t ball0, balln;
  uint32_t adj;
  uint32_t flags;
};
constexpr uint32_t BALL_MAX = 4096;
constexpr uint32_t SIG_BYTE_MAX = 120;

constexpr int kSymbolPlanesMaxA = 61;
__host__ __device__ inline void symbol_planes16(const uint8_t* row, uint32_t len, uint32_t (&w)[3]) {
  uint32_t p[6] = {0u, 0u, 0u, 0u, 0u, 0u};
  for (uint32_t i = 0; i < 16u && i < len; ++i) {
    const uint32_t v = (uint32_t)row[i] + 1u;
    for (uint32_t b = 0; b < 6u; ++b) p[b] |= ((v >> b) & 1u) << i;
  }
  w[0] = p[0] | p[1] << 16; w[1] = p[2] | p[3] << 16; w[2] = p[4] | p[5] << 16;
}

constexpr int NBITPLANES = 4;
constexpr uint32_t SCAN_TQ = 64;
constexpr uint32_t SCAN_TQ_DEFAULT = 48;
constexpr uint32_t SCAN_HITS = 512;
constexpr uint32_t SCAN_MASKW = 2048;
constexpr uint32_t SCAN_PBUF = 128;
constexpr uint32_t SCAN_CHUNK = 256;
constexpr uint32_t SCAN_CHUNK_FUSED = 128;
constexpr uint32_t SCAN_REGIONS = 64;
constexpr uint32_t RC_STRIDE = 32;
constexpr uint32_t RAW_INVALID = 0xFFFFFFFFu;
constexpr uint32_t RAW_ENTRY_MASK = 0x3FFFFFFFu;
constexpr uint32_t RAW_PREFILTERED = 0x40000000u;
constexpr uint32_t META_SKIPPED = 0xFFFFFFFFu;

struct EntRec {
  uint32_t vocab, freq, order, meta;
};

struct DevAlphabet {
  int16_t* fast = nullptr;
  uint32_t* coff = nullptr;
  uint4* cand = nullptr;
  uint8_t* bytes = nullptr;
  uint8_t* sym_group = nullptr;
  uint2* lower = nullptr;
  uint32_t nlower = 0;
  uint32_t* siglen_begin = nullptr;
};

struct BatchShell {
  hipEvent_t ev[6] = {};
  hipEvent_t ev_scan0 = nullptr, ev_fs0 = nullptr, ev_fs1 = nullptr, ev_done = nullptr, ev_in = nullptr;
  uint32_t* h_read = nullptr;
};
struct RunHints {
  std::mutex mu;
  bool valid = false;
  anx_threshold kth = {}, dth = {};
  double score_threshold = 0.0;
  int stop = 0;
  uint32_t seg = 0;
  double nq = 0, maxfill = 0, surv_fill = 0, list_fill = 0, total_surv = 0;
};
struct DeviceLexicon {
  int device = 0;
  int nplanes = 0;
  int nsym = 0;
  uint32_t nclasses = 0, nentries = 0, cstride = 0, max_len = 0;
  uint32_t* cls_planes = nullptr;
  uint32_t* cls_bits = nullptr;
  uint8_t* cls_len = nullptr;
  uint32_t* cls_off = nullptr;
  uint4* scan_rec = nullptr;
  uint2* scan_rec34 = nullptr;
  uint4* sig_e = nullptr;
  uint4* sighash = nullptr;
  uint4* sighash_e = nullptr;
  uint32_t hash_mask = 0;
  unsigned long long* ball = nullptr;
  uint32_t* ball_tab = nullptr;
  uint32_t ball_off[13] = {}, ball_n[13] = {};
  uint4* adj_hash = nullptr;
  uint32_t adj_mask = 0;
  uint32_t* adj_hdr = nullptr;
  uint2* adj_planes = nullptr;
  uint32_t* adj_ids = nullptr;
  uint32_t adj_nhdr = 0;
  mutable std::vector<AdjSlot> adj_hash_host;
  mutable std::vector<AdjHdr> adj_hdr_host;
// ... 152 lines not shown
```

analiticcl_amd/csrc/kernels_scan.hpp:

```cpp
#pragma once

enum { RC_RAW = 0, RC_VALID = 1, RC_FUSED = 2 , RC_TESTS = 4 ,
       RC_ADJ = 14 , RC_ADJ_FIRST = 15  };

struct WaveOut {
  uint32_t base, left;
  uint32_t emitted;
  uint32_t nbase;
  uint32_t split;
  uint32_t rbase, rend;
  uint32_t* ctr;
  uint32_t chunk;
};
__device__ inline uint32_t wave_inclusive_scan(uint32_t x) {
  uint32_t v = x;
  v += (uint32_t)__builtin_amdgcn_update_dpp(0, (int)x, 0x111, 0xF, 0xF, false);
  v += (uint32_t)__builtin_amdgcn_update_dpp(0, (int)x, 0x112, 0xF, 0xF, false);
  v += (uint32_t)__builtin_amdgcn_update_dpp(0, (int)x, 0x113, 0xF, 0xF, false);
  v += (uint32_t)__builtin_amdgcn_update_dpp(0, (int)v, 0x114, 0xF, 0xE, false);
  v += (uint32_t)__builtin_amdgcn_update_dpp(0, (int)v, 0x118, 0xF, 0xC, false);
  v += (uint32_t)__builtin_amdgcn_update_dpp(0, (int)v, 0x142, 0xA, 0xF, false);
  v += (uint32_t)__builtin_amdgcn_update_dpp(0, (int)v, 0x143, 0xC, 0xF, false);
  return v;
}
__device__ inline uint32_t wave_reserve(WaveOut& w, uint32_t ntot, uint32_t lane, uint32_t* total_out) {
  const uint32_t incl = wave_inclusive_scan(ntot);
  const uint32_t total = (uint32_t)__builtin_amdgcn_readlane((int)incl, 63);
  *total_out = total;
  w.split = w.left;
  if (total > w.left) {
    const uint32_t rest = total - w.left;
    const uint32_t need = rest > w.chunk ? rest : w.chunk;
    uint32_t b = 0;
    if (lane == 0) b = atomicAdd(&w.ctr[RC_RAW], need);
    w.nbase = w.rbase + __shfl(b, 0);
  }
  return incl - ntot;
}
__device__ inline void wave_reserve_total(WaveOut& w, uint32_t total, uint32_t lane) {
  w.split = w.left;
  if (total > w.left) {
    const uint32_t rest = total - w.left;
    const uint32_t need = rest > w.chunk ? rest : w.chunk;
    uint32_t b = 0;
    if (lane == 0) b = atomicAdd(&w.ctr[RC_RAW], need);
    w.nbase = w.rbase + (uint32_t)__builtin_amdgcn_readfirstlane((int)b);
  }
}
__device__ inline uint32_t wave_slot(const WaveOut& w, uint32_t g) {
  return g < w.split ? w.base + g : w.nbase + (g - w.split);
}
__device__ inline void wave_commit(WaveOut& w, uint32_t total) {
  if (total > w.left) {
    const uint32_t rest = total - w.left;
    const uint32_t need = rest > w.chunk ? rest : w.chunk;
    w.base = w.nbase + rest;
    w.left = need - rest;
  } else {
    w.base += total;
    w.left -= total;
  }
  w.emitted += total;
}
__device__ inline void wave_close(const WaveOut& w, uint32_t lane, uint2* __restrict__ raw) {
  for (uint32_t i = lane; i < w.left; i += 64)
    if (w.base + i < w.rend) raw[w.base + i] = make_uint2(RAW_INVALID, 0u);
  if (lane == 0 && w.emitted) atomicAdd(&w.ctr[RC_VALID], w.emitted);
}

struct ScanArgs {
  const Tile* tiles;
  uint32_t ntiles;
  const uint32_t* q_bits;
  const uint32_t* q_cv;
  const uint32_t* cls_bits;
  const uint32_t* cls_planes;
  const uint4* scan_rec;
  const uint2* scan_rec34;
  uint32_t pad_rec;
  uint32_t cstride;
  uint32_t pad_class;
  const uint8_t* cls_len;
  const uint32_t* cls_off;
  const uint4* sig;
  const uint4* sig_e;
  const uint4* sighash;
  const uint4* sighash_e;
  uint32_t hash_mask;
  const unsigned long long* ball;
  const uint32_t* adj_hdr;
  const uint2* adj_planes;
  const uint32_t* adj_ids;
  const uint32_t* sig_cbeg;
  uint2* raw;
  uint32_t region_cap;
  uint32_t chunk;
  uint32_t chunk_fused;
  uint32_t* rctr;
  const uint32_t* qexact;
  int want_exact;
  int drop_len;
  const uint4* q_rec;
  const uint4* e_rec;
  int fuse;
  uint32_t* qpairs;
  int dbg;
};

__device__ inline int32_t bcnt_acc(uint32_t x, int32_t acc) {
  int32_t r;
  asm("v_bcnt_u32_b32 %0, %1, %2" : "=v"(r) : "v"(x), "v"(acc));
  return r;
}
__device__ inline int32_t bcnt_acc_s(uint32_t x, int32_t acc) {
  int32_t r;
  asm("v_bcnt_u32_b32 %0, %1, %2" : "=v"(r) : "v"(x), "s"(acc));
  return r;
}

template <bool BITS, int NP, bool GEN, bool ADJ = false>
__device__ inline void scan_tile(const ScanArgs& AA, const Tile& t, uint32_t item, uint32_t* __restrict__ stage, uint32_t* __restrict__ hits,
                                 uint32_t* __restrict__ qlds, uint4* __restrict__ qsym, uint32_t* __restrict__ pbuf) {
  ScanArgs A = AA;
  if (!GEN) { A.want_exact = 0; A.qpairs = nullptr; A.drop_len = 1; A.qexact = nullptr; }
  constexpr int CPL = BITS ? 4 : (NP <= 8 ? 4 : NP <= 16 ? 2 : 1);
  constexpr int W = BITS ? NBITPLANES : NP;
  constexpr int QSTRIDE = BITS ? NBITPLANES : NP;
  constexpr uint32_t CHUNK = 64u * CPL;
  const uint32_t lane = threadIdx.x & 63;
  const uint32_t* __restrict__ cls_words = BITS ? A.cls_bits : A.cls_planes;
  const uint8_t* __restrict__ cls_len = A.cls_len;
  const uint32_t* __restrict__ cls_off = A.cls_off;
  uint2* __restrict__ raw = A.raw;
  const uint32_t cstride = A.cstride;
  const uint32_t region = item % SCAN_REGIONS;
  WaveOut wo{0, 0, 0, 0, 0, region * A.region_cap, (region + 1) * A.region_cap, A.rctr + region * RC_STRIDE, A.chunk};
  uint32_t ns = 0;
  uint32_t nchunks = 0;
  uint32_t arend = 0;
  int32_t alc[4] = {0, 0, 0, 0};
  uint2 apl[4] = {};
  uint32_t aid[4] = {};
  auto adj_load = [&](uint32_t row, uint2 (&pl)[4], uint32_t (&id)[4]) {
#pragma unroll
    for (int j = 0; j < 4; ++j) {
      pl[j] = make_uint2(0u, 0u);
      id[j] = A.pad_rec;
      if (row + (uint32_t)j < arend) {
        const size_t p = (size_t)(row + (uint32_t)j) * 64u + lane;
        pl[j] = A.adj_planes[p];
        id[j] = A.adj_ids[p];
      }
    }
  };
  {
    const uint32_t* __restrict__ src = (BITS ? A.q_bits : A.q_cv) + (size_t)t.q0 * QSTRIDE;
    for (uint32_t i = lane; i < t.nq * QSTRIDE; i += 64) qlds[i] = src[i];
  }
  const bool fuse = BITS && A.fuse && t.lq <= 16u && t.d <= 3u;
  if (fuse) wo.chunk = A.chunk_fused;
  if (BITS && fuse && lane < t.nq) qsym[lane] = rec32(A.q_rec, t.q0 + lane)[0];
  constexpr uint32_t PBUF = SCAN_PBUF;
  uint32_t nfused = 0;
  uint32_t npb = 0, phead = 0;

  uint32_t nhits = 0;
  uint32_t counted_only = 0;
  auto emit_dense = [&](bool fin) {
    while (npb >= 64u || (fin && npb)) {
      const uint32_t cnt = npb < 64u ? npb : 64u;
      const bool act = lane < cnt;
      const uint32_t pr = pbuf[(phead + lane) & (PBUF - 1u)];
      const uint32_t e = act ? (pr & 0x3FFFFFFu) : 0u, ql = act ? (pr >> 26) : 0u;
      bool keep = act;
      uint32_t flag = 0u;
      if (ANX_DBG(A.dbg) & 16) keep = false;
      if (BITS && fuse && !(ANX_DBG(A.dbg) & 16)) {
        nfused += cnt;
        const uint4 C = rec32(A.e_rec, e)[0];
        const int lc = (int)(rec32(A.e_rec, e)[1].x & 0xFFu), lq = (int)t.lq, d = (int)t.d;
        const uint4 Q = qsym[ql];
        const bool filt = act && lc <= 16;
        const int ml = lq > lc ? lq : lc;
        constexpr uint32_t M = 0x7F7F7F7Fu;
        bool rej;
        if (__any(filt && ml > 12)) {
          const uint32_t q4[4] = {Q.x & M, Q.y & M, Q.z & M, Q.w & M}, c6[6] = {M, C.x & M, C.y & M, C.z & M, C.w & M, M};
          rej = band_bound_rejects<4, true, true>(q4, c6, filt, d, lq, lc);
        } else if (__any(filt && ml > 8)) {
          const uint32_t q3[3] = {Q.x & M, Q.y & M, Q.z & M}, c5[5] = {M, C.x & M, C.y & M, C.z & M, M};
          rej = band_bound_rejects<3, true, true>(q3, c5, filt, d, lq, lc);
        } else {
          const uint32_t q2[2] = {Q.x & M, Q.y & M}, c4[4] = {M, C.x & M, C.y & M, M};
          rej = band_bound_rejects<2, true, true>(q2, c4, filt, d, lq, lc);
        }
        if (rej) { keep = false; ++counted_only; }
        if (filt) flag = RAW_PREFILTERED;
      }
      if (ANX_DBG(A.dbg) & 32) keep = false;
      const unsigned long long km = __ballot(keep);
      const uint32_t total = (uint32_t)__popcll(km);
      if (total) {
        wave_reserve_total(wo, total, lane);
        if (keep) {
          const uint32_t q = t.q0 + ql;
          uint32_t exact = 0u;
          if (A.want_exact) exact = A.qexact[q] == A.scan_rec[e].w ? 0x80000000u : 0u;
          const uint32_t g = __builtin_amdgcn_mbcnt_hi((uint32_t)(km >> 32), __builtin_amdgcn_mbcnt_lo((uint32_t)km, 0u));
          const uint32_t pos = wave_slot(wo, g);
          if (pos < wo.rend) raw[pos] = make_uint2(q, e | exact | flag);
        }
        wave_commit(wo, total);
      }
      phead = (phead + cnt) & (PBUF - 1u);
      npb -= cnt;
    }
  };
  auto flush = [&]() {
    for (uint32_t r0 = 0; r0 < nhits; r0 += 64) {
      const uint32_t idx = r0 + lane;
      uint32_t c = 0, m = 0, e0 = 0, ne = 0, qb = 0;
      if (idx < nhits) {
        bool count_only;
        if (BITS) {
          const uint32_t hx = reinterpret_cast<const uint16_t*>(hits + SCAN_HITS)[idx];
          m = hits[idx];
          qb = ((hx >> 8) & 1u) << 5;
          count_only = (hx >> 9) & 1u;
          e0 = stage[hx & 0xFFu];
          ne = 1;
          c = A.qpairs ? A.scan_rec[e0].w : 0u;
        } else {
          c = hits[2 * idx];
          m = hits[2 * idx + 1];
          qb = ((c >> 27) & 1u) << 5;
          c &= (1u << 27) - 1u;
          const uint32_t lc = cls_len[c];
          e0 = cls_off[c];
          ne = cls_off[c + 1] - e0;
          const uint32_t diff = lc > t.lq ? lc - t.lq : t.lq - lc;
          count_only = A.drop_len && diff > t.d;
        }
        if (A.qpairs) {
          for (uint32_t mm = m; mm; mm &= mm - 1u) {
            const uint32_t q = t.q0 + qb + (uint32_t)__ffs((int)mm) - 1u;
            if (!A.want_exact || A.qexact[q] == 0xFFFFFFFFu || A.qexact[q] == c) atomicAdd(&A.qpairs[q], ne);
          }
        }
        if (count_only) {
          counted_only += (uint32_t)__popc(m) * ne;
          m = 0;
        }
      }
      if (BITS) {
        while (true) {
          const bool has = m != 0u;
          const unsigned long long bm = __ballot(has);
          if (!bm) break;
          if (has) {
            const uint32_t bit = (uint32_t)__ffs((int)m) - 1u;
            m &= m - 1u;
            pbuf[(phead + npb + __builtin_amdgcn_mbcnt_hi((uint32_t)(bm >> 32), __builtin_amdgcn_mbcnt_lo((uint32_t)bm, 0u))) & (PBUF - 1u)] = e0 | ((qb + bit) << 26);
          }
          npb += (uint32_t)__popcll(bm);
          if (npb >= 64u) emit_dense(false);
        }
        continue;
      }
      uint32_t total;
      uint32_t g = wave_reserve(wo, (uint32_t)__popc(m) * ne, lane, &total);
      if (total <= wo.split && wo.base + total <= wo.rend) {
        uint2* __restrict__ dst = raw + wo.base;
        while (m) {
          const uint32_t bit = (uint32_t)__ffs((int)m) - 1u;
          m &= m - 1u;
          const uint32_t q = t.q0 + qb + bit;
          const uint32_t exact = (A.want_exact && A.qexact[q] == c) ? 0x80000000u : 0u;
          for (uint32_t i = 0; i < ne; ++i, ++g) dst[g] = make_uint2(q, (e0 + i) | exact);
        }
      } else {
        while (m) {
          const uint32_t bit = (uint32_t)__ffs((int)m) - 1u;
          m &= m - 1u;
          const uint32_t q = t.q0 + qb + bit;
          const uint32_t exact = (A.want_exact && A.qexact[q] == c) ? 0x80000000u : 0u;
          for (uint32_t i = 0; i < ne; ++i, ++g) {
            const uint32_t pos = wave_slot(wo, g);
            if (pos < wo.rend) raw[pos] = make_uint2(q, (e0 + i) | exact);
          }
        }
      }
      wave_commit(wo, total);
    }
    nhits = 0;
  };

  auto process = [&]() {
    ++nchunks;
    if (ANX_DBG(A.dbg) & 2) return;
    uint32_t cid[CPL], cw[CPL][W];
    int32_t thr[CPL];
    const bool need34 = BITS && ((t.kend >> 8) & 0xFFu) < t.nq;
#pragma unroll
    for (int j = 0; j < CPL; ++j) {
      const uint32_t idx = (uint32_t)j * 64u + lane;
      int32_t lc;
      if (ADJ) {
        const uint2 pl = apl[j];
        const uint32_t id = aid[j];
        stage[idx] = id;
        uint2 hi = make_uint2(0u, 0u);
        if (need34) hi = A.scan_rec34[id];
        cw[j][0] = pl.x; cw[j][1] = pl.y;
        if (W > 2) { cw[j][2] = hi.x; cw[j][W - 1] = hi.y; }
        lc = alc[j];
        const int32_t diff = lc > (int32_t)t.lq ? lc - (int32_t)t.lq : (int32_t)t.lq - lc;
        cid[j] = (A.drop_len && diff > (int32_t)t.d) ? id | (1u << 28) : id;
      } else {
      cid[j] = idx < ns ? stage[idx] : (BITS ? A.pad_rec : A.pad_class);
      if (BITS) {
        const uint4 mt = A.scan_rec[cid[j]];
        uint2 hi = make_uint2(0u, 0u);
        if (need34) hi = A.scan_rec34[cid[j]];
        const uint32_t plw[4] = {mt.x, mt.y, hi.x, hi.y};
#pragma unroll
        for (int p = 0; p < W; ++p) cw[j][p] = plw[p];
        lc = (int32_t)mt.z;
        const int32_t diff = lc > (int32_t)t.lq ? lc - (int32_t)t.lq : (int32_t)t.lq - lc;
        if (A.drop_len && diff > (int32_t)t.d) cid[j] |= 1u << 28;
      } else {
#pragma unroll
        for (int p = 0; p < W; ++p) cw[j][p] = cls_words[(size_t)p * cstride + cid[j]];
        lc = (int32_t)cls_len[cid[j]];
      }
      }
      if (BITS) {
        const int32_t need = ((int32_t)t.lq - (int32_t)t.k + lc + 1) >> 1;
        thr[j] = -(need < 1 ? 1 : need);
      } else {
        const int32_t share = (int32_t)t.lq + lc - 1;
        thr[j] = share < (int32_t)t.k ? share : (int32_t)t.k;
      }
    }
    for (uint32_t qb = 0; qb < t.nq; qb += 32) {
      const uint32_t npass = (ANX_DBG(A.dbg) & 1) ? 1u : (t.nq - qb < 32u ? t.nq - qb : 32u);
      uint32_t hm[CPL];
#pragma unroll
      for (int j = 0; j < CPL; ++j) hm[j] = 0xFFFFFFFFu;
      auto test_query = [&](auto tw, uint32_t qi) {
        constexpr int TW = decltype(tw)::value;
        uint32_t qreg[TW];
#pragma unroll
        for (int p = 0; p < TW; ++p) qreg[p] = qlds[(qb + qi) * QSTRIDE + p];
#pragma unroll
        for (int j = 0; j < CPL; ++j) {
          int32_t acc;
          if (BITS) {
            acc = ADJ ? bcnt_acc_s(qreg[0] & cw[j][0], thr[j]) : bcnt_acc(qreg[0] & cw[j][0], thr[j]);
#pragma unroll
            for (int p = 1; p < TW; ++p) acc = bcnt_acc(qreg[p] & cw[j][p], acc);
          } else {
            uint32_t sad = 0;
#pragma unroll
            for (int p = 0; p < TW; ++p) sad = __builtin_amdgcn_sad_u8(qreg[p], cw[j][p], sad);
            acc = thr[j] - (int32_t)sad;
          }
          hm[j] = __builtin_amdgcn_alignbit(hm[j], (uint32_t)acc, 31);
        }
      };
      auto run_queries = [&](auto tw, uint32_t lo, uint32_t hi) {
        uint32_t qi = lo;
        for (; qi + 2 <= hi; qi += 2) {
          test_query(tw, qi);
          test_query(tw, qi + 1);
        }
        if (qi < hi) test_query(tw, qi);
      };
      if (BITS) {
        const uint32_t pend = qb + npass;
        auto clampr = [&](uint32_t x) { return (x < qb ? qb : (x > pend ? pend : x)) - qb; };
        const uint32_t b1 = clampr(t.kend & 0xFFu), b2 = clampr((t.kend >> 8) & 0xFFu), b3 = clampr((t.kend >> 16) & 0xFFu);
        run_queries(std::integral_constant<int, 1>{}, 0u, b1);
        run_queries(std::integral_constant<int, 2>{}, b1, b2);
        run_queries(std::integral_constant<int, 3>{}, b2, b3);
        run_queries(std::integral_constant<int, BITS ? 4 : 1>{}, b3, npass);
      } else {
        run_queries(std::integral_constant<int, BITS ? 1 : NP>{}, 0u, npass);
      }
      const uint32_t valid = npass >= 32u ? 0xFFFFFFFFu : ((1u << npass) - 1u);
      uint32_t any = 0;
#pragma unroll
      for (int j = 0; j < CPL; ++j) {
        hm[j] = ~hm[j] & valid;
        any |= hm[j];
      }
      if (__ballot(any != 0) == 0ull || (ANX_DBG(A.dbg) & 8)) continue;
#pragma unroll
      for (int j = 0; j < CPL; ++j) {
        const bool nz = hm[j] != 0;
        const unsigned long long bm = __ballot(nz);
        const uint32_t cnt = (uint32_t)__popcll(bm);
        if (cnt) {
          if (nz) {
            const uint32_t pos = nhits + __builtin_amdgcn_mbcnt_hi((uint32_t)(bm >> 32), __builtin_amdgcn_mbcnt_lo((uint32_t)bm, 0u));
            const uint32_t hmask = __brev(hm[j]) >> (32u - npass);
            if (BITS) {
              hits[pos] = hmask;
              reinterpret_cast<uint16_t*>(hits + SCAN_HITS)[pos] = (uint16_t)(((uint32_t)j * 64u + lane) | ((qb >> 5) << 8) | (((cid[j] >> 28) & 1u) << 9));
            } else {
              hits[2 * pos] = cid[j] | ((qb >> 5) << 27);
              hits[2 * pos + 1] = hmask;
            }
          }
          nhits += cnt;
        }
      }
      if (!BITS && nhits > SCAN_HITS - CHUNK) flush();
    }
    if (BITS) flush();
  };

  uint32_t* __restrict__ sdelta = stage + CHUNK;
  uint32_t* __restrict__ smask = stage + CHUNK + 64;
  auto stage_runs = [&](bool ok, uint32_t cb, uint32_t n) {
    ok = ok && n != 0u;
    const unsigned long long okm = __ballot(ok);
    if (!okm || (ANX_DBG(A.dbg) & 4)) return;
    const uint32_t cnt = ok ? n : 0u;
    const uint32_t incl = wave_inclusive_scan(cnt);
    const uint32_t carry = ns & 63u;
    const uint32_t total = carry + (uint32_t)__builtin_amdgcn_readlane((int)incl, 63);
    uint32_t wbase = ns - carry;
    const uint32_t endp = carry + incl - 1u;
    if (ok) sdelta[__builtin_amdgcn_mbcnt_hi((uint32_t)(okm >> 32), __builtin_amdgcn_mbcnt_lo((uint32_t)okm, 0u))] = cb + cnt - 1u - endp;
    uint32_t rbase = 0;
    for (uint32_t w0 = 0; w0 < total; w0 += SCAN_MASKW) {
      if (lane < SCAN_MASKW / 32u) smask[lane] = 0u;
      if (ok && endp - w0 < SCAN_MASKW) atomicOr(smask + ((endp - w0) >> 5), 1u << (endp & 31u));
      const uint32_t wend = total < w0 + SCAN_MASKW ? total : w0 + SCAN_MASKW;
      for (uint32_t p0 = w0; p0 < wend; p0 += 64) {
        const uint32_t mlo = (uint32_t)__builtin_amdgcn_readfirstlane((int)smask[((p0 - w0) >> 6) * 2u]), mhi = (uint32_t)__builtin_amdgcn_readfirstlane((int)smask[((p0 - w0) >> 6) * 2u + 1u]);
        const uint32_t r = rbase + __builtin_amdgcn_mbcnt_hi(mhi, __builtin_amdgcn_mbcnt_lo(mlo, 0u));
        rbase += (uint32_t)__popc(mlo) + (uint32_t)__popc(mhi);
        const uint32_t p = p0 + lane;
        const uint32_t id = sdelta[r & 63u] + p;
        if (p >= carry && p < total) stage[wbase + lane] = id;
        if (p0 + 64u <= total) {
          wbase += 64u;
          ns = wbase;
          if (wbase == CHUNK) {
            process();
            ns = 0;
            wbase = 0;
          }
        } else {
          ns = wbase + (total - p0);
        }
      }
    }
  };
  const uint4* __restrict__ sigtab = BITS ? A.sig_e : A.sig;
  if (ADJ) {
    const cptr_u32 hp = (cptr_u32)(A.adj_hdr + (size_t)(t.adj - 1u) * 8u);
    const uint32_t row0 = hp[0], c0 = hp[1], c1 = hp[2], c2 = hp[3], c3 = hp[4], c4 = hp[5], c5 = hp[6], c6 = hp[7];
    uint32_t rbeg = t.k >= 3u ? 0u : t.k == 2u ? c0 : t.k == 1u ? c1 : c2;
    uint32_t rend = t.k >= 3u ? c6 : t.k == 2u ? c5 : t.k == 1u ? c4 : c3;
    if (t.flags & 2u) { rbeg = t.s0; rend = t.s1; }
    arend = row0 + rend;
    if (lane == 0 && rend > rbeg) {
      atomicAdd(&wo.ctr[RC_ADJ], rend - rbeg);
      if (t.flags & 1u) atomicAdd(&wo.ctr[RC_ADJ_FIRST], rend - rbeg);
    }
    uint2 npl[4];
    uint32_t nid[4];
    if (rbeg < rend) adj_load(row0 + rbeg, npl, nid);
    for (uint32_t r = rbeg; r < rend; r += (uint32_t)CPL) {
#pragma unroll
      for (int j = 0; j < 4; ++j) {
        const uint32_t rr = r + (uint32_t)j;
        alc[j] = (int32_t)t.lq - 3 + (int32_t)((rr >= c0) + (rr >= c1) + (rr >= c2) + (rr >= c3) + (rr >= c4) + (rr >= c5));
        apl[j] = npl[j];
        aid[j] = nid[j];
      }
      if (r + (uint32_t)CPL < rend) adj_load(row0 + r + (uint32_t)CPL, npl, nid);
      process();
    }
  } else if (t.balln) {
    const unsigned long long H = 0x8080808080808080ull;
    const unsigned long long sq = (unsigned long long)t.sig_lo | (unsigned long long)t.sig_hi << 32;
    const uint4* __restrict__ htab = BITS ? A.sighash_e : A.sighash;
    for (uint32_t base = 0; base < t.balln; base += 64) {
      const uint32_t i = base + lane;
      bool found = false;
      uint32_t first = 0, count = 0;
      if (i < t.balln) {
        const unsigned long long dl = A.ball[t.ball0 + i];
        const unsigned long long r = ((sq & ~H) + (dl & ~H)) ^ ((sq ^ dl) & H);
        if (!(r & (r << 1) & H)) {
          const uint32_t lo = (uint32_t)r, hi = (uint32_t)(r >> 32);
          uint32_t h = sig_hash(lo, hi) & A.hash_mask;
          for (int p = 0; p < 17; ++p) {
            const uint4 e = htab[h];
            if (!e.w) break;
            if (e.x == lo && e.y == hi) { found = true; first = e.z; count = e.w; break; }
            h = (h + 1u) & A.hash_mask;
          }
        }
      }
      stage_runs(found, first, count);
    }
  } else {
    const uint4* __restrict__ sigp = sigtab + t.s0 + lane;
    uint4 sg_next = t.s0 < t.s1 ? *sigp : make_uint4(0xFFFFFFFFu, 0xFFFFFFFFu, 0u, 0u);
    for (uint32_t sb = t.s0; sb < t.s1; sb += 64) {
      const uint4 sg = sg_next;
      sigp += 64;
      if (sb + 64 < t.s1) sg_next = *sigp;
      const bool ok = __builtin_amdgcn_sad_u8(sg.x, t.sig_lo, __builtin_amdgcn_sad_u8(sg.y, t.sig_hi, 0u)) <= t.k;
      stage_runs(ok, sg.z, sg.w);
    }
  }
  if (!ADJ && ns) process();
  flush();
  if (BITS) emit_dense(true);
  if (A.drop_len) {
    const uint32_t tot = (uint32_t)__builtin_amdgcn_readlane((int)wave_inclusive_scan(counted_only), 63);
    wo.emitted += tot;
  }
  wave_close(wo, lane, raw);
  if (BITS && lane == 0 && nfused) atomicAdd(&wo.ctr[RC_FUSED], nfused);
  if (lane == 0 && nchunks) {
    if (BITS) {
      const uint32_t e[5] = {0u, t.kend & 0xFFu, (t.kend >> 8) & 0xFFu, (t.kend >> 16) & 0xFFu, t.nq};
      for (int k = 1; k <= NBITPLANES; ++k)
        if (e[k] > e[k - 1])
          atomicAdd(reinterpret_cast<unsigned long long*>(wo.ctr + RC_TESTS + 2 * k), (unsigned long long)nchunks * CHUNK * (e[k] - e[k - 1]));
    } else {
      atomicAdd(reinterpret_cast<unsigned long long*>(wo.ctr + RC_TESTS), (unsigned long long)nchunks * CHUNK * t.nq);
    }
  }
}

constexpr uint32_t SCAN_STAGE = 64 * 4 + 64 + SCAN_MASKW / 32;
template <int NP, bool BITS, bool GEN, bool ADJ = false>
__device__ inline void scan_wave(const ScanArgs& A) {
  constexpr int QWORDS = SCAN_TQ * (BITS ? NBITPLANES : NP);
  __shared__ uint32_t s_qlds[4][QWORDS];
  __shared__ __attribute__((aligned(16))) uint32_t s_stage[4][ADJ ? 64 * 4 : SCAN_STAGE];
  __shared__ uint32_t s_hits[4][BITS ? SCAN_HITS + SCAN_HITS / 2 : 2 * SCAN_HITS];
  __shared__ uint4 s_qsym[BITS ? 4 : 1][BITS ? SCAN_TQ : 1];
  __shared__ uint32_t s_pbuf[BITS ? 4 : 1][BITS ? SCAN_PBUF : 1];
  const uint32_t wid = threadIdx.x >> 6;
  const uint32_t item = (uint32_t)__builtin_amdgcn_readfirstlane((int)(blockIdx.x * 4u + wid));
  if (item >= A.ntiles) return;
  const cptr_u32 tp = (cptr_u32)(A.tiles + item);
  Tile t;
  t.q0 = tp[0]; t.nq = tp[1]; t.s0 = tp[2]; t.s1 = tp[3]; t.k = tp[4]; t.lq = tp[5]; t.sig_lo = tp[6]; t.sig_hi = tp[7]; t.kind = tp[8]; t.d = tp[9]; t.kend = tp[10]; t.ball0 = tp[11]; t.balln = tp[12]; t.adj = tp[13]; t.flags = tp[14];
  scan_tile<BITS, NP, GEN, ADJ>(A, t, item, s_stage[wid], s_hits[wid], s_qlds[wid], s_qsym[BITS ? wid : 0], s_pbuf[BITS ? wid : 0]);
}
template <bool GEN>
__global__ __launch_bounds__(256) __attribute__((amdgpu_waves_per_eu(5, 8))) void k_scan_bits(ScanArgs A) { scan_wave<8, true, GEN>(A); }
template <bool GEN>
__global__ __launch_bounds__(256) __attribute__((amdgpu_waves_per_eu(6, 8))) void k_scan_adj(ScanArgs A) { scan_wave<8, true, GEN, true>(A); }
template <int NP>
__global__ __launch_bounds__(256) void k_scan_sad(ScanArgs A) { scan_wave<NP, false, true>(A); }


template <int NP>
__global__ __launch_bounds__(256) void k_scan_small(ScanArgs A) {
  constexpr int QW = NP > NBITPLANES ? NP : NBITPLANES;
  __shared__ uint32_t s_qlds[4][QW];
  __shared__ __attribute__((aligned(16))) uint32_t s_stage[4][SCAN_STAGE];
  __shared__ uint32_t s_hits[4][2 * SCAN_HITS];
  __shared__ uint4 s_qsym[4][1];
  __shared__ uint32_t s_pbuf[4][SCAN_PBUF];
  const uint32_t wid = threadIdx.x >> 6;
  const uint32_t item = (uint32_t)__builtin_amdgcn_readfirstlane((int)(blockIdx.x * 4u + wid));
  if (item >= A.ntiles) return;
  const cptr_u32 tp = (cptr_u32)(A.tiles + item);
  Tile t;
  t.q0 = tp[0]; t.nq = tp[1]; t.s0 = tp[2]; t.s1 = tp[3]; t.k = tp[4]; t.lq = tp[5]; t.sig_lo = tp[6]; t.sig_hi = tp[7]; t.kind = tp[8]; t.d = tp[9]; t.kend = tp[10]; t.ball0 = tp[11]; t.balln = tp[12]; t.adj = tp[13]; t.flags = tp[14];
  if (t.nq == 0u) return;
  if (t.kind == 0u) scan_tile<false, NP, true>(A, t, item, s_stage[wid], s_hits[wid], s_qlds[wid], s_qsym[wid], s_pbuf[wid]);
  else if (t.adj) scan_tile<true, 8, false, true>(A, t, item, s_stage[wid], s_hits[wid], s_qlds[wid], s_qsym[wid], s_pbuf[wid]);
  else scan_tile<true, 8, false>(A, t, item, s_stage[wid], s_hits[wid], s_qlds[wid], s_qsym[wid], s_pbuf[wid]);
}
```

analiticcl_amd/csrc/small_path.hpp:

```cpp
#pragma once

constexpr uint32_t SMALL_MAX_BYTES = 64;
constexpr uint32_t SMALL_SHIFT = 15;
constexpr uint32_t SMALL_SURV_CAP = 16384;
constexpr uint32_t SMALL_LIST_BLOCKS = 2;
constexpr uint32_t SMALL_FS_BLK = 512;
constexpr uint32_t SMALL_FETCH_BLOCKS = 8;
constexpr uint32_t SMALL_ROWS_PER_Q = 16;

struct SmallCtx {
  int device = 0;
  hipStream_t st = nullptr;
  char* h_in = nullptr;
  char* h_out = nullptr;
  SmallEnc enc;
  uint32_t *counters = nullptr, *rctr = nullptr, *sctr = nullptr, *lctr = nullptr, *qsurv = nullptr, *soff = nullptr, *qcur = nullptr, *qmaxfreq = nullptr, *qexpand = nullptr,
           *r_count = nullptr;
  uint2* raw = nullptr;
  SurvRec* surv = nullptr;
  uint32_t *list8 = nullptr, *listg = nullptr, *listw = nullptr;
  SurvRow* c_rows = nullptr;
  DevRow* r_rows = nullptr;
  double* t_key = nullptr;
  FsCold* d_cold = nullptr;
// ... 52 lines not shown
  if (small_iota(e.perm, SMALL_MAX, c->st) != ANX_OK || hipStreamSynchronize(c->st) != hipSuccess) { err = "small path: set-up kernel"; return nullptr; }
  return c.release();
}
static SmallCtx* small_ctx_acquire(const DeviceLexicon* dl, std::string& err) {
  DevPool& pl = pool_of(dl->device);
  {
    std::lock_guard<std::mutex> g(pl.mu);
    if (!pl.small_idle.empty()) { SmallCtx* c = pl.small_idle.back(); pl.small_idle.pop_back(); return c; }
  }
  return small_ctx_create(dl, err);
}
static void small_ctx_release(SmallCtx* c) {
  DevPool& pl = pool_of(c->device);
  std::lock_guard<std::mutex> g(pl.mu);
  pl.small_idle.push_back(c);
}
static void small_ctxs_destroy(int device) {
  DevPool& pl = pool_of(device);
  std::vector<SmallCtx*> drop;
  { std::lock_guard<std::mutex> g(pl.mu); drop.swap(pl.small_idle); }
  for (SmallCtx* c : drop) small_ctx_destroy(c);
}

static std::atomic<uint64_t> g_small_taken{0}, g_small_overflow{0};
void small_stats(uint64_t* out) { out[0] = g_small_taken.load(); out[1] = g_small_overflow.load(); }

int small_find(const HostModel& m, const DeviceLexicon* dl, const char* const* utf8, size_t n, const anx_params& p, anx_result** out_rows, size_t** out_offs,
               std::string& err) {
  if (!dl || n == 0 || n > SMALL_MAX || !switches().small_path || dl->any_variants || p.stop_at_exact_match || dl->nplanes > 42) return 1;
  uint32_t lens[SMALL_MAX];
  uint32_t maxbytes = 0;
  for (size_t i = 0; i < n; ++i) {
    const size_t l = utf8[i] ? strlen(utf8[i]) : 0;
    if (l > SMALL_MAX_BYTES) return 1;
    lens[i] = (uint32_t)l;
    maxbytes = std::max(maxbytes, (uint32_t)l);
  }
  if (hipSetDevice(dl->device) != hipSuccess) { err = "hipSetDevice failed"; return ANX_ENODEVICE; }
  SmallCtx* c = small_ctx_acquire(dl, err);
  if (!c) { (void)hipGetLastError(); return 1; }
  struct Release { SmallCtx* c; ~Release() { small_ctx_release(c); } } rel{c};
  hipStream_t st = c->st;
  uint32_t* h_off = reinterpret_cast<uint32_t*>(c->h_in + SMALL_IN_BLOB);
  {
    size_t pos = 0;
    for (size_t i = 0; i < n; ++i) {
      h_off[i] = (uint32_t)pos;
      if (lens[i]) memcpy(c->h_in + pos, utf8[i], lens[i]);
      c->h_in[pos + lens[i]] = '\0';
      pos += (size_t)lens[i] + 1;
    }
    h_off[n] = (uint32_t)pos;
    memset(c->h_in + pos, 0, 16);
  }
  const uint32_t n32 = (uint32_t)n;
  const uint32_t qw = std::max<uint32_t>(1u, (maxbytes + 15u) / 16u);
  const uint32_t d = (uint32_t)clamp_threshold(p.max_edit_distance, (int)maxbytes, kMaxEditDistance);
  const size_t row_cap = std::min<size_t>(c->row_cap, n * (size_t)SMALL_ROWS_PER_Q + 64);
  anx_result* rows = static_cast<anx_result*>(host_result_alloc(row_cap * sizeof(anx_result)));
  if (!rows) return 1;
  if (!host_result_is_pinned(rows)) { host_result_free(rows); return 1; }
  SmallCtl* h_ctl = reinterpret_cast<SmallCtl*>(c->h_out);
  unsigned long long* h_off64 = reinterpret_cast<unsigned long long*>(c->h_out + 64);
  h_ctl->rows = 0xFFFFFFFEu;
  SmallZero z{};
  {
    uint32_t* zp[8] = {c->counters, c->rctr, c->sctr, c->lctr, c->qsurv, c->qmaxfreq, c->qexpand, nullptr};
    const uint32_t zn[8] = {CTR_N, SCAN_REGIONS * RC_STRIDE, SCAN_REGIONS * RC_STRIDE, 3 * SCAN_REGIONS * RC_STRIDE, n32, n32, n32, 0u};
    for (int i = 0; i < 8; ++i) { z.p[i] = zp[i]; z.n[i] = zn[i]; }
  }
  const uint8_t* in_blob = reinterpret_cast<const uint8_t*>(c->h_in);
  const uint32_t* in_off = h_off;
  const uint32_t slots = n32 <= 128u ? 32u : n32 <= 512u ? 16u : 8u;
  int rc = small_encode_launch(m, dl, c->enc, in_blob, in_off, n32, qw, p, z, slots, true, h_off, st, err);
  if (rc) { host_result_free(rows); return rc; }
  const uint32_t region_cap = 1u << SMALL_SHIFT;
  {
    ScanArgs A;
    A.tiles = c->enc.tiles; A.ntiles = slots * n32; A.q_bits = c->enc.q_bits; A.q_cv = c->enc.q_cv;
    A.cls_bits = dl->cls_bits; A.cls_planes = dl->cls_planes; A.scan_rec = dl->scan_rec; A.scan_rec34 = dl->scan_rec34; A.pad_rec = dl->nentries; A.cstride = dl->cstride; A.pad_class = dl->nclasses;
    A.cls_len = dl->cls_len; A.cls_off = dl->cls_off; A.sig = dl->sig; A.sig_e = dl->sig_e; A.sig_cbeg = dl->sig_cbeg; A.sighash = dl->sighash; A.sighash_e = dl->sighash_e; A.hash_mask = dl->hash_mask; A.ball = dl->ball;
    A.adj_hdr = dl->adj_hdr; A.adj_planes = dl->adj_planes; A.adj_ids = dl->adj_ids;
    A.chunk = 64; A.chunk_fused = 32;
    A.raw = c->raw; A.region_cap = region_cap; A.rctr = c->rctr; A.qexact = c->enc.qexact; A.want_exact = 0; A.drop_len = 1;
    A.q_rec = c->enc.q_rec; A.e_rec = dl->e_rec;

    A.fuse = (switches().fuse_prefilter && switches().prefilter) ? 1 : 0;
    A.qpairs = nullptr; A.dbg = 0;
    const dim3 grid((A.ntiles + 3) / 4);
    switch (dl->nplanes) {
      case 8: hipLaunchKernelGGL(k_scan_small<8>, grid, dim3(256), 0, st, A); break;
      case 16: hipLaunchKernelGGL(k_scan_small<16>, grid, dim3(256), 0, st, A); break;
      case 24: hipLaunchKernelGGL(k_scan_small<24>, grid, dim3(256), 0, st, A); break;
      case 32: hipLaunchKernelGGL(k_scan_small<32>, grid, dim3(256), 0, st, A); break;
      default: hipLaunchKernelGGL(k_scan_small<42>, grid, dim3(256), 0, st, A); break;
    }
  }
  ScoreArgs sa;
  sa.dbg = 0;
  sa.quot = dl->quot;
  sa.store_pairs = 0;
  sa.w_ld = m.weights.ld; sa.w_lcs = m.weights.lcs; sa.w_prefix = m.weights.prefix; sa.w_suffix = m.weights.suffix; sa.w_case = m.weights.casew;
  sa.w_sum = m.weights.ld + m.weights.lcs + m.weights.prefix + m.weights.suffix + m.weights.casew;
  sa.score_threshold = p.score_threshold;
  sa.have_freq = m.have_freq ? 1 : 0;
  sa.any_variants = 0;
  sa.lqp = qw * 16;
  sa.lcp = (dl->max_len + 15) / 16 * 16;
  uint32_t stride = sa.lqp + sa.lcp + (d + 2) * (2 * d + 3);
  stride = (stride + 3) / 4;
  if ((stride & 1) == 0) stride++;
  sa.stride = stride * 4;
  sa.qw = qw;
  uint32_t threads = 256;
  while (threads > 64 && (size_t)threads * sa.stride > 64 * 1024) threads >>= 1;
  if ((size_t)threads * sa.stride > 64 * 1024) { host_result_free(rows); (void)hipStreamSynchronize(st); return 1; }
  const SurvOut so{c->surv, c->sctr, SMALL_SURV_CAP, nullptr, 0u};
  const bool have_long_q = qw > 1;
  const int enable_filter = switches().prefilter, enable_fast = switches().score_fast;
  const int fastD = (enable_fast && d >= 1 && d <= 3) ? (int)d : 0;
  const SlotList l8{c->list8, c->lctr, SMALL_SURV_CAP}, lg{c->listg, c->lctr + SCAN_REGIONS * RC_STRIDE, SMALL_SURV_CAP}, lw{c->listw, c->lctr + 2 * SCAN_REGIONS * RC_STRIDE, SMALL_SURV_CAP};
  const PairArgs pa{c->raw, c->enc.q_meta, c->enc.q_rows, c->enc.q_rec, dl->e_rec, dl->ent_meta, dl->ent_rowoff, dl->rows, dl->ent_freq, dl->ent_var_off,
                    nullptr, nullptr, c->qmaxfreq, c->qsurv, c->qexpand, dl->e_planes};
  uint32_t fs_cap = 2048;
  while (fs_cap < region_cap && fs_cap < n32 * 12u + 2048u) fs_cap *= 2u;
  FilterArgs fa;
  fa.region_shift = SMALL_SHIFT; fa.rctr = c->rctr; fa.qexact = c->enc.qexact; fa.stop = 0; fa.enable = enable_filter;
  const bool use8 = fastD > 0 && threads == 256;
  fa.use_nw8 = (have_long_q || use8) ? 1 : 0; fa.counters = c->counters; fa.stat_ctr = c->sctr; fa.fill_cap = fs_cap; fa.blk = SMALL_FS_BLK;
  {
    const double key[12] = {sa.w_ld, sa.w_lcs, sa.w_prefix, sa.w_suffix, sa.w_case, sa.w_sum, sa.score_threshold, (double)sa.have_freq, (double)sa.lqp, (double)sa.lcp, (double)sa.stride,
                            (double)sa.qw + 1e3 * (double)(reinterpret_cast<uintptr_t>(sa.quot) & 0xFFFFFFFFu)};
    if (!c->cold_valid || memcmp(key, c->cold_key, sizeof key) != 0) {
      memcpy(c->cold_key, key, sizeof key);
      c->h_cold_last = FsCold{sa, so, l8, lg, lw};
      if (hipMemcpyAsync(c->d_cold, &c->h_cold_last, sizeof(FsCold), hipMemcpyHostToDevice, st) != hipSuccess || hipStreamSynchronize(st) != hipSuccess) {
        host_result_free(rows);
        err = "small path: argument upload";
        return ANX_ENODEVICE;
      }
      c->cold_valid = true;
    }
  }
  const dim3 fgrid(((fs_cap + SMALL_FS_BLK - 1) / SMALL_FS_BLK) * SCAN_REGIONS);
  const bool split_wide = switches().fs_split != 0;
  const bool b7 = switches().fs_b7 && m.alphabet.size() + 1 < 0x7E;
  const bool planes = b7 && switches().fs_planes && (int)m.alphabet.size() <= kSymbolPlanesMaxA;
#define ANX_FS_LAUNCH(DD, WW, BB) hipLaunchKernelGGL((k_filter_score<DD, WW, BB>), fgrid, dim3(256), 0, st, fa, pa, static_cast<const FsCold*>(c->d_cold))
#define ANX_FS_PICK(WW, BB)                        \
  do {                                             \
    if (fastD == 1) ANX_FS_LAUNCH(1, WW, BB);      \
    else if (fastD == 2) ANX_FS_LAUNCH(2, WW, BB); \
    else if (fastD == 3) ANX_FS_LAUNCH(3, WW, BB); \
    else ANX_FS_LAUNCH(0, WW, BB);                 \
  } while (0)
  if (split_wide) { if (planes) ANX_FS_PICK(false, 2); else if (b7) ANX_FS_PICK(false, 1); else ANX_FS_PICK(false, 0); }
  else { if (b7) ANX_FS_PICK(true, 1); else ANX_FS_PICK(true, 0); }
#undef ANX_FS_PICK
#undef ANX_FS_LAUNCH
  if (threads == 256) {
    SmallListArgs L{lw, l8, lg, (split_wide && enable_filter) ? 1 : 0, (fastD && (have_long_q || use8)) ? 1 : 0, fastD};
    const dim3 lgrid(SCAN_REGIONS);
    const size_t dyn = (size_t)threads * sa.stride;
    if (fastD == 1) hipLaunchKernelGGL(k_small_lists<1>, lgrid, dim3(256), dyn, st, L, fa, pa, sa, so);
    else if (fastD == 2) hipLaunchKernelGGL(k_small_lists<2>, lgrid, dim3(256), dyn, st, L, fa, pa, sa, so);
    else if (fastD == 3) hipLaunchKernelGGL(k_small_lists<3>, lgrid, dim3(256), dyn, st, L, fa, pa, sa, so);
    else hipLaunchKernelGGL(k_small_lists<0>, lgrid, dim3(256), dyn, st, L, fa, pa, sa, so);
// ... 44 lines not shown
```

include/anx.h:

```cpp
#ifndef ANX_H
#define ANX_H
#include <stddef.h>
#include <stdint.h>
#ifdef __cplusplus
extern "C" {
#endif

#define ANX_ABI_VERSION 3

enum {
  ANX_OK = 0,
  ANX_EINVAL = -1,
  ANX_EIO = -2,
  ANX_ENOTBUILT = -3,
  ANX_ENODEVICE = -4,
  ANX_ELIMIT = -5,
  ANX_EEMPTY = -6
};

typedef struct anx_model anx_model;
typedef struct anx_batch anx_batch;

typedef struct anx_weights {
  double ld, lcs, prefix, suffix, casew;
// ... 74 lines not shown
const char *anx_model_lexicon_name(const anx_model *, uint64_t i);
int anx_model_to_device(anx_model *, int device);
int anx_model_to_devices(anx_model *, const int *devices, int n);
int anx_model_num_replicas(const anx_model *);
int anx_model_replica_device(const anx_model *, int replica);
int anx_model_has(const anx_model *, const char *utf8);
uint64_t anx_model_vocab_size(const anx_model *);
const char *anx_model_vocab_text(const anx_model *, uint64_t vocab_id);
uint32_t anx_model_vocab_frequency(const anx_model *, uint64_t vocab_id);
uint32_t anx_model_vocab_lexindex(const anx_model *, uint64_t vocab_id);
uint64_t anx_model_num_instances(const anx_model *);
uint64_t anx_model_num_classes(const anx_model *);
uint64_t anx_model_bucket_size(const anx_model *, int charcount);
int anx_model_alphabet_size(const anx_model *);
int anx_model_normalize(const anx_model *, const char *utf8, uint8_t *out, int cap);
int anx_model_anahash(const anx_model *, const char *utf8, char *out, int cap);

int anx_find_variants_batch(const anx_model *, const char *const *utf8, size_t n, const anx_params *,
                            anx_result **out_rows, size_t **out_offsets);
void anx_results_free(anx_result *rows, size_t *offsets);

anx_batch *anx_batch_encode(const anx_model *, const char *const *utf8, size_t n, const anx_params *);
anx_batch *anx_batch_encode_packed(const anx_model *, const char *blob, size_t blob_len, size_t n, const anx_params *);
anx_batch *anx_batch_encode_packed_device(const anx_model *, const void *device_blob, size_t blob_len, size_t n, const anx_params *);
anx_batch *anx_batch_encode_packed_device_on(const anx_model *, const void *device_blob, size_t blob_len, size_t n, const anx_params *, void *stream);
int anx_batch_run(const anx_model *, anx_batch *, void *stream);
int anx_batch_run_async(const anx_model *, anx_batch *, void *stream);
int anx_batch_wait(const anx_model *, anx_batch *);
int anx_batch_fetch(const anx_batch *, anx_result **out_rows, size_t **out_offsets);
int anx_batch_fetch_compact(const anx_batch *, anx_topk_record **out_rows, uint32_t **out_offsets);
void anx_compact_free(anx_topk_record *rows, uint32_t *offsets);
void anx_compact_to_results(const anx_topk_record *rows, size_t n_rows, anx_result *out);
typedef struct anx_pipeline anx_pipeline;
anx_pipeline *anx_pipeline_new(const anx_model *, int depth );
int anx_pipeline_submit_packed(anx_pipeline *, const char *blob, size_t blob_len, size_t n, const anx_params *);
int anx_pipeline_pending(const anx_pipeline *);
int anx_pipeline_next(anx_pipeline *, anx_topk_record **out_rows, uint32_t **out_offsets, size_t *out_n);
void anx_pipeline_free(anx_pipeline *);
int anx_batch_fetch_pairs(const anx_batch *, anx_pair **out_pairs, size_t *out_n);
void anx_pairs_free(anx_pair *);
int anx_batch_pair_counts(anx_batch *, uint32_t **out_counts);
void anx_counts_free(uint32_t *);
int anx_batch_export_topk(const anx_batch *, void *device_dst, uint32_t stride, void *stream);
int anx_batch_export_compact(const anx_batch *, void *device_dst, size_t capacity, void *stream, size_t *used);
int anx_batch_gather_compact(const anx_batch *, int dst_device, void *device_dst, size_t capacity, size_t *shard_offsets, size_t *used);
typedef struct anx_batch_stats {
  uint64_t n_queries;
  uint64_t n_pairs;
  uint64_t n_class_tests;
  uint64_t n_results;
  uint64_t n_scan_blocks;
  uint64_t n_tests_kind[5];
  uint64_t n_pair_slots;
  uint64_t n_survivors;
  float ms_scan, ms_group, ms_score, ms_rank, ms_total;
  float ms_scan_kernel;
  uint64_t n_selected;
  float ms_filter_score_kernel;
  uint64_t n_prefiltered_in_scan;
  uint64_t n_conf_scripts;
  uint64_t n_adj_tiles;
  uint64_t n_adj_records;
  uint64_t n_adj_records_first;
} anx_batch_stats;
int anx_batch_get_stats(const anx_batch *, anx_batch_stats *, size_t struct_size);
int anx_batch_num_shards(const anx_batch *);
int anx_batch_shard_info(const anx_batch *, int shard, int *device, size_t *first_input, size_t *n_inputs);
int anx_batch_shard_inputs(const anx_batch *, int shard, const uint32_t **indices);
void anx_batch_free(anx_batch *);
void anx_device_pool_trim(int device);
void anx_shutdown(void);

int anx_debug_set_switch(const char *name, const char *value);
void anx_debug_kernel_timer(int enable);
int anx_debug_kernel_time(const char *name, double *total_ms, uint64_t *launches);
int anx_debug_search_stats(uint64_t out[4]);
int anx_debug_small_stats(uint64_t out[2]);
int anx_debug_length_split(const anx_model *, const char *const *utf8, size_t n, const anx_params *, int n_shards, uint8_t *out_shard,
                           const double *learn_ms);
int anx_debug_signature(const anx_model *, const char *utf8, uint64_t *out_sig);
int anx_debug_entries(const anx_model *, uint32_t **out_vocab_ids, size_t *n);
int anx_debug_adjacency(const anx_model *, int closure, uint64_t budget_bytes, const uint64_t *sigs, size_t n, uint32_t *out_cum,
                        uint32_t **out_ids, uint64_t *out_stats);
int anx_debug_adjacency_device(const anx_model *, const uint64_t *sigs, size_t n, uint32_t *out_cum, uint32_t **out_ids);
int anx_debug_band_bound(int device, const uint8_t *q_rows, const uint8_t *c_rows, const uint8_t *lq, const uint8_t *lc, size_t n,
                         int d, int form, uint8_t *out_reject);

int anx_format_query_output(const anx_model *, const char *const *utf8_inputs, size_t n, const anx_result *rows,
                            const size_t *offsets, float freq_weight, int json, int output_lexmatch,
                            uint64_t first_seqnr, char **out, size_t *out_len);
void anx_string_free(char *);

int anx_model_add_to_confusables(anx_model *, const char *editscript, double weight);
int anx_model_read_confusablelist(anx_model *, const char *path);
void anx_model_set_confusables_before_pruning(anx_model *);
int anx_edit_script(const char *source, const char *target, char *out, int cap);
int anx_model_confusable_weight(const anx_model *, const char *input_utf8, uint64_t vocab_id, double *out_weight);

typedef struct anx_search_params {
  anx_params base;
  uint8_t max_ngram;
  uint32_t max_seq;
  float lm_weight;
  float variantmodel_weight;
  float contextrules_weight;
  int32_t unicodeoffsets;
} anx_search_params;
typedef struct anx_match {
  uint64_t begin, end;
  uint32_t n;
  int32_t selected;
  uint64_t var_begin, var_end;
  uint32_t tag_begin, tag_end;
} anx_match;
typedef struct anx_match_tag {
  uint16_t tag;
  uint8_t seqnr;
  uint8_t pad_;
} anx_match_tag;
void anx_default_search_params(anx_search_params *);
int anx_find_all_matches_batch(const anx_model *, const char *const *utf8_texts, size_t n, const anx_search_params *,
                               anx_match **out_matches, size_t **out_offsets, anx_result **out_rows, size_t *out_n_rows,
                               anx_match_tag **out_tags);
void anx_matches_free(anx_match *matches, size_t *offsets, anx_result *rows, anx_match_tag *tags);
int anx_format_search_output(const anx_model *, const char *const *utf8_texts, size_t n, const anx_match *matches,
                             const size_t *offsets, const anx_result *rows, const anx_match_tag *tags,
                             float freq_weight, int json, int output_lexmatch, uint64_t first_seqnr, char **out,
                             size_t *out_len);

int anx_model_add_contextrule(anx_model *, const char *pattern, float score, const char *const *tags, size_t n_tags,
                              const char *const *tagoffsets, size_t n_tagoffsets);
int anx_model_read_contextrules(anx_model *, const char *path);
size_t anx_model_num_tags(const anx_model *);
const char *anx_model_tag_name(const anx_model *, size_t index);

int anx_learn_variants(anx_model *, const char *const *utf8, size_t n, const anx_params *, int auto_build, uint64_t *count);
int anx_learn_variants_search(anx_model *, const char *const *utf8_texts, size_t n, const anx_search_params *, int auto_build,
                              uint64_t *count);
int anx_learn_apply_rows(anx_model *, const char *const *utf8, size_t n, const anx_result *rows, const size_t *offsets, uint64_t *count);
int64_t anx_model_variants(const anx_model *, uint64_t vocab_id, uint8_t *kinds, uint64_t *ids, double *scores, size_t cap);
uint32_t anx_model_vocab_type(const anx_model *, uint64_t vocab_id);
int anx_format_variant_list(const anx_model *, int json, char **out);
int anx_debug_learn_stats(uint64_t out[4]);
int anx_debug_learn_times(double out[6]);

#ifdef __cplusplus
}
#endif
#endif
```

Measured before the change: 53.91 billion.

## Resolve adjacency row ranges into tiles and count length-rejected rows without emitting hits

Tile construction now precomputes the absolute adjacency row range and the six packed section boundaries into the tile record, which grows to 16 words. The scan kernel then skips the dependent header load per tile. A second switch bit lets length-rejected adjacency candidates be tallied as counted-only instead of being written to the hit buffer. This trades a larger tile record and 16-bit section limits (with a fallback) for fewer global loads and less hit traffic.

```diff
diff --git a/analiticcl_amd/_lib.py b/analiticcl_amd/_lib.py
--- a/analiticcl_amd/_lib.py
+++ b/analiticcl_amd/_lib.py
@@ -198,6 +198,7 @@
         "anx_debug_entries": (C.c_int, [vp, C.POINTER(C.POINTER(C.c_uint32)), C.POINTER(C.c_size_t)]),
         "anx_debug_adjacency": (C.c_int, [vp, C.c_int, C.c_uint64, vp, C.c_size_t, vp, C.POINTER(C.POINTER(C.c_uint32)), vp]),
         "anx_debug_adjacency_device": (C.c_int, [vp, vp, C.c_size_t, vp, C.POINTER(C.POINTER(C.c_uint32))]),
+        "anx_debug_adj_tile_rows": (C.c_int, [vp, C.c_uint32, vp]),
         "anx_debug_band_bound": (C.c_int, [C.c_int, vp, vp, vp, vp, C.c_size_t, C.c_int, C.c_int, vp]),
         "anx_batch_free": (None, [vp]),
         "anx_device_pool_trim": (None, [C.c_int]),
diff --git a/analiticcl_amd/csrc/adjacency.h b/analiticcl_amd/csrc/adjacency.h
--- a/analiticcl_amd/csrc/adjacency.h
+++ b/analiticcl_amd/csrc/adjacency.h
@@ -2,6 +2,8 @@
 #include <cstdint>
 #include <cstddef>
 #include <vector>
+
+#include "sig_hash.h"
 
 namespace anx {
 
@@ -16,6 +18,27 @@
   uint32_t row0;
   uint32_t cum[kAdjSections];
 };
+ANX_HOST_DEVICE inline void adj_rows_for_k(const uint32_t* hdr, uint32_t k, uint32_t& b, uint32_t& e) {
+  b = k >= 3u ? 0u : hdr[3u - k];
+  e = k >= 3u ? hdr[7] : hdr[4u + k];
+}
+struct AdjTileRows { uint32_t beg, end, sec[3]; };
+ANX_HOST_DEVICE inline bool adj_tile_rows(const uint32_t* hdr, uint32_t b, uint32_t e, AdjTileRows& r) {
+  static_assert(kAdjSections == 7, "six section boundaries, three words");
+  const uint32_t n = e > b ? e - b : 0u;
+  if (n > 0xFFFFu) return false;
+  r.beg = hdr[0] + b;
+  r.end = r.beg + n;
+  for (int i = 0; i < 3; ++i) {
+    uint32_t w[2];
+    for (int h = 0; h < 2; ++h) {
+      const uint32_t c = hdr[1 + 2 * i + h];
+      w[h] = c <= b ? 0u : (c - b < n ? c - b : n);
+    }
+    r.sec[i] = w[0] | w[1] << 16;
+  }
+  return true;
+}
 struct AdjSlot {
   uint32_t lo, hi;
   uint32_t hdr1;
diff --git a/analiticcl_amd/csrc/capi.cpp b/analiticcl_amd/csrc/capi.cpp
--- a/analiticcl_amd/csrc/capi.cpp
+++ b/analiticcl_amd/csrc/capi.cpp
@@ -398,6 +398,15 @@
   *out_ids = ids;
   return ANX_OK;
 }
+int anx_debug_adj_tile_rows(const uint32_t* hdr, uint32_t k, uint32_t* out) {
+  if (!hdr || !out) return fail(ANX_EINVAL, "NULL argument");
+  if (k > (uint32_t)anx::kAdjRadius) return fail(ANX_EINVAL, "k > 3 has no list rows");
+  anx::adj_rows_for_k(hdr, k, out[0], out[1]);
+  anx::AdjTileRows r;
+  if (!anx::adj_tile_rows(hdr, out[0], out[1], r)) return fail(ANX_ELIMIT, "more rows than the section boundaries address");
+  out[2] = r.beg; out[3] = r.end; out[4] = r.sec[0]; out[5] = r.sec[1]; out[6] = r.sec[2];
+  return ANX_OK;
+}
 int anx_debug_adjacency_device(const anx_model* m, const uint64_t* sigs, size_t n, uint32_t* out_cum, uint32_t** out_ids) {
   if (!m || (!sigs && n) || (!out_cum && n) || !out_ids) return fail(ANX_EINVAL, "NULL argument");
   if (m->replicas.empty()) return fail(ANX_ENODEVICE, "model is not resident on a device");
diff --git a/analiticcl_amd/csrc/encode.hip b/analiticcl_amd/csrc/encode.hip
--- a/analiticcl_amd/csrc/encode.hip
+++ b/analiticcl_amd/csrc/encode.hip
@@ -401,6 +401,8 @@
   int probe;
   const uint4* adj_hash;
   uint32_t adj_mask;
+  const uint32_t* adj_hdr;
+  int tile_rows;
 };
 __device__ inline uint32_t adj_lookup(const uint4* tab, uint32_t mask, uint32_t lo, uint32_t hi, uint32_t* rows) {
   if (!mask) return 0u;
@@ -482,7 +484,13 @@
     Tile tl;
     tl.q0 = s; tl.nq = tn; tl.s0 = a0; tl.s1 = a1; tl.k = k; tl.lq = lq; tl.sig_lo = (uint32_t)sig; tl.sig_hi = (uint32_t)(sig >> 32);
     tl.kind = sad ? 0u : 1u; tl.d = d; tl.kend = sad ? 0u : (ke[0] | ke[1] << 8 | ke[2] << 16);
-    tl.ball0 = ball0; tl.balln = balln; tl.adj = adj; tl.flags = (s == hs && part == 0u) ? 1u : 0u;
+    tl.ball0 = ball0; tl.balln = balln; tl.adj = adj; tl.flags = (s == hs && part == 0u) ? 1u : 0u; tl.sec45 = 0u;
+    if (adj && (t.tile_rows & 1)) {
+      const uint32_t* hp = t.adj_hdr + (size_t)(adj - 1u) * 8u;
+      uint32_t rb, re;
+      adj_rows_for_k(hp, k, rb, re);
+      tile_resolve_rows(tl, hp, rb, re);
+    }
     t.tiles[base + part] = tl;
     const unsigned long long cost = adj ? (unsigned long long)adj_rows * (8u + tn) + 16u : (unsigned long long)tn * (a1 - a0 + 64u);
     t.tkey[base + part] = (sad ? 0x80000000u : adj ? 0u : 0x40000000u) | (0x3FFFFFFFu - (uint32_t)(cost < 0x3FFFFFFFull ? cost : 0x3FFFFFFFull));
@@ -495,7 +503,7 @@
   if (i < n && tiles[i].adj && (i + 1 == n || !tiles[i + 1].adj)) ctr[5] = i + 1u;
 }
 
-__global__ __launch_bounds__(256) void k_small_tiles(GatherArgs g, TileArgs t, SmallZero z, uint32_t slots, const uint32_t* __restrict__ adj_hdr) {
+__global__ __launch_bounds__(256) void k_small_tiles(GatherArgs g, TileArgs t, SmallZero z, uint32_t slots) {
   const uint32_t s = blockIdx.x * 256 + threadIdx.x, nthreads = gridDim.x * 256u;
 #pragma unroll
   for (int a = 0; a < 8; ++a)
@@ -515,10 +523,10 @@
     uint32_t adj_rows = 0;
     const uint32_t adj = (!sad && k <= (uint32_t)kAdjRadius) ? adj_lookup(t.adj_hash, t.adj_mask, (uint32_t)sig, (uint32_t)(sig >> 32), &adj_rows) : 0u;
     uint32_t rbeg = 0, rend = 0;
+    const uint32_t* hp = nullptr;
     if (adj) {
-      const uint32_t* hp = adj_hdr + (size_t)(adj - 1u) * 8u;
-      rbeg = k >= 3u ? 0u : k == 2u ? hp[1] : k == 1u ? hp[2] : hp[3];
-      rend = k >= 3u ? hp[7] : k == 2u ? hp[6] : k == 1u ? hp[5] : hp[4];
+      hp = t.adj_hdr + (size_t)(adj - 1u) * 8u;
+      adj_rows_for_k(hp, k, rbeg, rend);
       const uint32_t rows = rend > rbeg ? rend - rbeg : 0u;
       nparts = min(slots, max(1u, rows / 8u));
       step = ((rows + nparts - 1u) / nparts + 3u) & ~3u;
@@ -529,12 +537,13 @@
       tl.q0 = s; tl.nq = 1u; tl.s0 = a0; tl.s1 = a1; tl.k = k; tl.lq = lq; tl.sig_lo = (uint32_t)sig; tl.sig_hi = (uint32_t)(sig >> 32);
       tl.kind = sad ? 0u : 1u; tl.d = d;
       tl.kend = sad ? 0u : ((kind <= 1u ? 1u : 0u) | (kind <= 2u ? 1u : 0u) << 8 | (kind <= 3u ? 1u : 0u) << 16);
-      tl.ball0 = ball0; tl.balln = balln; tl.adj = adj; tl.flags = part == 0u ? 1u : 0u;
+      tl.ball0 = ball0; tl.balln = balln; tl.adj = adj; tl.flags = part == 0u ? 1u : 0u; tl.sec45 = 0u;
       if (adj) {
         tl.s0 = min(rend, rbeg + part * step);
         tl.s1 = min(rend, tl.s0 + step);
         tl.flags |= 2u;
         if (tl.s0 >= tl.s1 && part) tl.nq = 0u;
+        if (t.tile_rows & 1) tile_resolve_rows(tl, hp, tl.s0, tl.s1);
       }
       t.tiles[(size_t)part * t.nq + s] = tl;
     }
@@ -569,8 +578,9 @@
   ta.tq = 1; ta.nq = n; ta.q_meta = e.q_meta; ta.s_kind = e.s_kind; ta.s_sig = e.s_sig; ta.siglen_begin = dl->alpha.siglen_begin; ta.ctr = nullptr;
   ta.ball_tab = dl->ball_tab; ta.probe = probe_enabled() ? 1 : 0;
   ta.adj_hash = dl->adj_hash; ta.adj_mask = switches().scan_adj ? dl->adj_mask : 0u;
+  ta.adj_hdr = dl->adj_hdr; ta.tile_rows = switches().scan_tile_rows;
   ta.head = nullptr; ta.tcount = nullptr; ta.tiles = e.tiles; ta.tkey = nullptr;
-  hipLaunchKernelGGL(k_small_tiles, gn, dim3(256), 0, st, ga, ta, z, slots, dl->adj_hdr);
+  hipLaunchKernelGGL(k_small_tiles, gn, dim3(256), 0, st, ga, ta, z, slots);
   HIP_TRY(hipGetLastError());
   return ANX_OK;
 }
@@ -739,6 +749,7 @@
   ta.nq = nq; ta.q_meta = b->q_meta; ta.s_kind = s_kind; ta.s_sig = s_sig; ta.siglen_begin = dl->alpha.siglen_begin; ta.ctr = d_ctr;
   ta.ball_tab = dl->ball_tab; ta.probe = probe_enabled() ? 1 : 0;
   ta.adj_hash = dl->adj_hash; ta.adj_mask = switches().scan_adj ? dl->adj_mask : 0u;
+  ta.adj_hdr = dl->adj_hdr; ta.tile_rows = switches().scan_tile_rows;
   uint32_t *d_head = nullptr, *d_tcount = nullptr;
   if ((rc = sc.get(&d_head, nq, err)) || (rc = sc.get(&d_tcount, (size_t)nq + 1, err))) return rc;
   ta.head = d_head; ta.tcount = d_tcount; ta.tiles = nullptr; ta.tkey = nullptr;
diff --git a/analiticcl_amd/csrc/engine.hip b/analiticcl_amd/csrc/engine.hip
--- a/analiticcl_amd/csrc/engine.hip
+++ b/analiticcl_amd/csrc/engine.hip
@@ -826,8 +826,17 @@
       for (uint32_t part = 0; part < nsplit; ++part) {
         const uint32_t a0 = s0 + part * step, a1 = std::min(s1, a0 + step);
         if (a0 >= a1 && part) break;
-        b->tiles.push_back(Tile{(uint32_t)s, tn, a0, a1, k, lq, (uint32_t)h_sig[i], (uint32_t)(h_sig[i] >> 32), sad ? 0u : 1u,
-                                (h_meta[i] >> 16) & 0xFFu, kend, ball0, balln, adj, (s == i && part == 0u) ? 1u : 0u});
+        Tile tl{};
+        tl.q0 = (uint32_t)s; tl.nq = tn; tl.s0 = a0; tl.s1 = a1; tl.k = k; tl.lq = lq; tl.sig_lo = (uint32_t)h_sig[i]; tl.sig_hi = (uint32_t)(h_sig[i] >> 32);
+        tl.kind = sad ? 0u : 1u; tl.d = (h_meta[i] >> 16) & 0xFFu; tl.kend = kend; tl.ball0 = ball0; tl.balln = balln; tl.adj = adj;
+        tl.flags = (s == i && part == 0u) ? 1u : 0u;
+        if (adj && (switches().scan_tile_rows & 1)) {
+          const uint32_t* hp = reinterpret_cast<const uint32_t*>(&dl->adj_hdr_host[adj - 1]);
+          uint32_t rb, re;
+          adj_rows_for_k(hp, k, rb, re);
+          tile_resolve_rows(tl, hp, rb, re);
+        }
+        b->tiles.push_back(tl);
       }
     }
     i = j;
@@ -1254,6 +1263,7 @@
       HIP_TRY(hipMemsetAsync(b->qpairs, 0, nq * sizeof(uint32_t), st));
       A.qpairs = b->qpairs;
     }
+    A.tile_rows = switches().scan_tile_rows;
     A.dbg = 0;
 #ifdef ANX_DEBUG_SWITCHES
     { const char* e = getenv("ANX_SCAN_DBG"); A.dbg = e ? atoi(e) : 0; }
diff --git a/analiticcl_amd/csrc/host_model.cpp b/analiticcl_amd/csrc/host_model.cpp
--- a/analiticcl_amd/csrc/host_model.cpp
+++ b/analiticcl_amd/csrc/host_model.cpp
@@ -521,6 +521,7 @@
     {"ANX_SCAN_WALK", [](Switches& s, const char* v) { s.scan_walk_flat = v && strcmp(v, "flat") == 0; }},
     {"ANX_SCAN_TQ", [](Switches& s, const char* v) { const int x = v ? atoi(v) : 0; s.scan_tq = x >= 1 && x <= 64 ? x : 0; }},
     {"ANX_SCAN_ADJ", [](Switches& s, const char* v) { s.scan_adj = flag01(v, 1); }},
+    {"ANX_SCAN_TILE_ROWS", [](Switches& s, const char* v) { const int x = v ? atoi(v) : 3; s.scan_tile_rows = x >= 0 && x <= 3 ? x : 3; }},
     {"ANX_ADJ_BUILD", [](Switches& s, const char* v) { s.adj_build_host = v && strcmp(v, "host") == 0; }},
     {"ANX_ADJ_CLOSURE", [](Switches& s, const char* v) { const int x = v ? atoi(v) : 2; s.adj_closure = x >= 0 && x <= kAdjMaxClosure ? x : kAdjMaxClosure; }},
     {"ANX_SCAN_CHUNK_FUSED", [](Switches& s, const char* v) { const int x = v ? atoi(v) : 0; s.scan_chunk_fused = x >= 32 && x <= 1024 ? x : 0; }},
diff --git a/analiticcl_amd/csrc/host_model.h b/analiticcl_amd/csrc/host_model.h
--- a/analiticcl_amd/csrc/host_model.h
+++ b/analiticcl_amd/csrc/host_model.h
@@ -55,6 +55,7 @@
   int scan_walk_flat = 0;
   int scan_tq = 0;
   int scan_adj = 1;
+  int scan_tile_rows = 3;
   int adj_build_host = 0;
   int adj_closure = 2;
   long adj_budget_mb = 16384;
diff --git a/analiticcl_amd/csrc/kernels_common.hpp b/analiticcl_amd/csrc/kernels_common.hpp
--- a/analiticcl_amd/csrc/kernels_common.hpp
+++ b/analiticcl_amd/csrc/kernels_common.hpp
@@ -9,10 +9,20 @@
   uint32_t kind;
   uint32_t d;
   uint32_t kend;
-  uint32_t ball0, balln;
+  union { uint32_t ball0; uint32_t sec01; };
+  union { uint32_t balln; uint32_t sec23; };
   uint32_t adj;
   uint32_t flags;
-};
+  uint32_t sec45;
+};
+static_assert(sizeof(Tile) == 16 * sizeof(uint32_t), "one scalar load per tile");
+__host__ __device__ inline void tile_resolve_rows(Tile& tl, const uint32_t* hdr, uint32_t b, uint32_t e) {
+  AdjTileRows r;
+  if (!adj_tile_rows(hdr, b, e, r)) return;
+  tl.s0 = r.beg; tl.s1 = r.end;
+  tl.sec01 = r.sec[0]; tl.sec23 = r.sec[1]; tl.sec45 = r.sec[2];
+  tl.flags |= 4u;
+}
 constexpr uint32_t BALL_MAX = 4096;
 constexpr uint32_t SIG_BYTE_MAX = 120;
 
diff --git a/analiticcl_amd/csrc/kernels_scan.hpp b/analiticcl_amd/csrc/kernels_scan.hpp
--- a/analiticcl_amd/csrc/kernels_scan.hpp
+++ b/analiticcl_amd/csrc/kernels_scan.hpp
@@ -104,6 +104,7 @@
   const uint4* e_rec;
   int fuse;
   uint32_t* qpairs;
+  int tile_rows;
   int dbg;
 };
 
@@ -139,6 +140,7 @@
   uint32_t nchunks = 0;
   uint32_t arend = 0;
   int32_t alc[4] = {0, 0, 0, 0};
+  const bool co_rows = !GEN && ADJ && (A.tile_rows & 2);
   uint2 apl[4] = {};
   uint32_t aid[4] = {};
   auto adj_load = [&](uint32_t row, uint2 (&pl)[4], uint32_t (&id)[4]) {
@@ -300,6 +302,7 @@
     if (ANX_DBG(A.dbg) & 2) return;
     uint32_t cid[CPL], cw[CPL][W];
     int32_t thr[CPL];
+    uint32_t rco = 0;
     const bool need34 = BITS && ((t.kend >> 8) & 0xFFu) < t.nq;
 #pragma unroll
     for (int j = 0; j < CPL; ++j) {
@@ -315,7 +318,8 @@
         if (W > 2) { cw[j][2] = hi.x; cw[j][W - 1] = hi.y; }
         lc = alc[j];
         const int32_t diff = lc > (int32_t)t.lq ? lc - (int32_t)t.lq : (int32_t)t.lq - lc;
-        cid[j] = (A.drop_len && diff > (int32_t)t.d) ? id | (1u << 28) : id;
+        if (A.drop_len && diff > (int32_t)t.d) rco |= 1u << j;
+        cid[j] = id;
       } else {
       cid[j] = idx < ns ? stage[idx] : (BITS ? A.pad_rec : A.pad_class);
       if (BITS) {
@@ -392,6 +396,10 @@
 #pragma unroll
       for (int j = 0; j < CPL; ++j) {
         hm[j] = ~hm[j] & valid;
+        if (co_rows && ((rco >> j) & 1u)) {
+          counted_only = (uint32_t)bcnt_acc(hm[j], (int32_t)counted_only);
+          hm[j] = 0u;
+        }
         any |= hm[j];
       }
       if (__ballot(any != 0) == 0ull || (ANX_DBG(A.dbg) & 8)) continue;
@@ -406,7 +414,7 @@
             const uint32_t hmask = __brev(hm[j]) >> (32u - npass);
             if (BITS) {
               hits[pos] = hmask;
-              reinterpret_cast<uint16_t*>(hits + SCAN_HITS)[pos] = (uint16_t)(((uint32_t)j * 64u + lane) | ((qb >> 5) << 8) | (((cid[j] >> 28) & 1u) << 9));
+              reinterpret_cast<uint16_t*>(hits + SCAN_HITS)[pos] = (uint16_t)(((uint32_t)j * 64u + lane) | ((qb >> 5) << 8) | (((ADJ ? (rco >> j) : (cid[j] >> 28)) & 1u) << 9));
             } else {
               hits[2 * pos] = cid[j] | ((qb >> 5) << 27);
               hits[2 * pos + 1] = hmask;
@@ -461,28 +469,38 @@
   };
   const uint4* __restrict__ sigtab = BITS ? A.sig_e : A.sig;
   if (ADJ) {
-    const cptr_u32 hp = (cptr_u32)(A.adj_hdr + (size_t)(t.adj - 1u) * 8u);
-    const uint32_t row0 = hp[0], c0 = hp[1], c1 = hp[2], c2 = hp[3], c3 = hp[4], c4 = hp[5], c5 = hp[6], c6 = hp[7];
-    uint32_t rbeg = t.k >= 3u ? 0u : t.k == 2u ? c0 : t.k == 1u ? c1 : c2;
-    uint32_t rend = t.k >= 3u ? c6 : t.k == 2u ? c5 : t.k == 1u ? c4 : c3;
-    if (t.flags & 2u) { rbeg = t.s0; rend = t.s1; }
-    arend = row0 + rend;
-    if (lane == 0 && rend > rbeg) {
-      atomicAdd(&wo.ctr[RC_ADJ], rend - rbeg);
-      if (t.flags & 1u) atomicAdd(&wo.ctr[RC_ADJ_FIRST], rend - rbeg);
+    uint32_t abeg, aend, b0, b1, b2, b3, b4, b5;
+    if (t.flags & 4u) {
+      abeg = t.s0; aend = t.s1;
+      b0 = abeg + (t.sec01 & 0xFFFFu); b1 = abeg + (t.sec01 >> 16);
+      b2 = abeg + (t.sec23 & 0xFFFFu); b3 = abeg + (t.sec23 >> 16);
+      b4 = abeg + (t.sec45 & 0xFFFFu); b5 = abeg + (t.sec45 >> 16);
+    } else {
+      const cptr_u32 hp = (cptr_u32)(A.adj_hdr + (size_t)(t.adj - 1u) * 8u);
+      const uint32_t row0 = hp[0], c0 = hp[1], c1 = hp[2], c2 = hp[3], c3 = hp[4], c4 = hp[5], c5 = hp[6], c6 = hp[7];
+      uint32_t rbeg = t.k >= 3u ? 0u : t.k == 2u ? c0 : t.k == 1u ? c1 : c2;
+      uint32_t rend = t.k >= 3u ? c6 : t.k == 2u ? c5 : t.k == 1u ? c4 : c3;
+      if (t.flags & 2u) { rbeg = t.s0; rend = t.s1; }
+      abeg = row0 + rbeg; aend = row0 + (rend > rbeg ? rend : rbeg);
+      b0 = row0 + c0; b1 = row0 + c1; b2 = row0 + c2; b3 = row0 + c3; b4 = row0 + c4; b5 = row0 + c5;
+    }
+    arend = aend;
+    if (lane == 0 && aend > abeg) {
+      atomicAdd(&wo.ctr[RC_ADJ], aend - abeg);
+      if (t.flags & 1u) atomicAdd(&wo.ctr[RC_ADJ_FIRST], aend - abeg);
     }
     uint2 npl[4];
     uint32_t nid[4];
-    if (rbeg < rend) adj_load(row0 + rbeg, npl, nid);
-    for (uint32_t r = rbeg; r < rend; r += (uint32_t)CPL) {
+    if (abeg < aend) adj_load(abeg, npl, nid);
+    for (uint32_t r = abeg; r < aend; r += (uint32_t)CPL) {
 #pragma unroll
       for (int j = 0; j < 4; ++j) {
         const uint32_t rr = r + (uint32_t)j;
-        alc[j] = (int32_t)t.lq - 3 + (int32_t)((rr >= c0) + (rr >= c1) + (rr >= c2) + (rr >= c3) + (rr >= c4) + (rr >= c5));
+        alc[j] = (int32_t)t.lq - 3 + (int32_t)((rr >= b0) + (rr >= b1) + (rr >= b2) + (rr >= b3) + (rr >= b4) + (rr >= b5));
         apl[j] = npl[j];
         aid[j] = nid[j];
       }
-      if (r + (uint32_t)CPL < rend) adj_load(row0 + r + (uint32_t)CPL, npl, nid);
+      if (r + (uint32_t)CPL < aend) adj_load(r + (uint32_t)CPL, npl, nid);
       process();
     }
   } else if (t.balln) {
@@ -555,7 +573,7 @@
   if (item >= A.ntiles) return;
   const cptr_u32 tp = (cptr_u32)(A.tiles + item);
   Tile t;
-  t.q0 = tp[0]; t.nq = tp[1]; t.s0 = tp[2]; t.s1 = tp[3]; t.k = tp[4]; t.lq = tp[5]; t.sig_lo = tp[6]; t.sig_hi = tp[7]; t.kind = tp[8]; t.d = tp[9]; t.kend = tp[10]; t.ball0 = tp[11]; t.balln = tp[12]; t.adj = tp[13]; t.flags = tp[14];
+  t.q0 = tp[0]; t.nq = tp[1]; t.s0 = tp[2]; t.s1 = tp[3]; t.k = tp[4]; t.lq = tp[5]; t.sig_lo = tp[6]; t.sig_hi = tp[7]; t.kind = tp[8]; t.d = tp[9]; t.kend = tp[10]; t.ball0 = tp[11]; t.balln = tp[12]; t.adj = tp[13]; t.flags = tp[14]; t.sec45 = tp[15];
   scan_tile<BITS, NP, GEN, ADJ>(A, t, item, s_stage[wid], s_hits[wid], s_qlds[wid], s_qsym[BITS ? wid : 0], s_pbuf[BITS ? wid : 0]);
 }
 template <bool GEN>
@@ -579,7 +597,7 @@
   if (item >= A.ntiles) return;
   const cptr_u32 tp = (cptr_u32)(A.tiles + item);
   Tile t;
-  t.q0 = tp[0]; t.nq = tp[1]; t.s0 = tp[2]; t.s1 = tp[3]; t.k = tp[4]; t.lq = tp[5]; t.sig_lo = tp[6]; t.sig_hi = tp[7]; t.kind = tp[8]; t.d = tp[9]; t.kend = tp[10]; t.ball0 = tp[11]; t.balln = tp[12]; t.adj = tp[13]; t.flags = tp[14];
+  t.q0 = tp[0]; t.nq = tp[1]; t.s0 = tp[2]; t.s1 = tp[3]; t.k = tp[4]; t.lq = tp[5]; t.sig_lo = tp[6]; t.sig_hi = tp[7]; t.kind = tp[8]; t.d = tp[9]; t.kend = tp[10]; t.ball0 = tp[11]; t.balln = tp[12]; t.adj = tp[13]; t.flags = tp[14]; t.sec45 = tp[15];
   if (t.nq == 0u) return;
   if (t.kind == 0u) scan_tile<false, NP, true>(A, t, item, s_stage[wid], s_hits[wid], s_qlds[wid], s_qsym[wid], s_pbuf[wid]);
   else if (t.adj) scan_tile<true, 8, false, true>(A, t, item, s_stage[wid], s_hits[wid], s_qlds[wid], s_qsym[wid], s_pbuf[wid]);
diff --git a/analiticcl_amd/csrc/small_path.hpp b/analiticcl_amd/csrc/small_path.hpp
--- a/analiticcl_amd/csrc/small_path.hpp
+++ b/analiticcl_amd/csrc/small_path.hpp
@@ -158,7 +158,7 @@
     A.cls_len = dl->cls_len; A.cls_off = dl->cls_off; A.sig = dl->sig; A.sig_e = dl->sig_e; A.sig_cbeg = dl->sig_cbeg; A.sighash = dl->sighash; A.sighash_e = dl->sighash_e; A.hash_mask = dl->hash_mask; A.ball = dl->ball;
     A.adj_hdr = dl->adj_hdr; A.adj_planes = dl->adj_planes; A.adj_ids = dl->adj_ids;
     A.chunk = 64; A.chunk_fused = 32;
-    A.raw = c->raw; A.region_cap = region_cap; A.rctr = c->rctr; A.qexact = c->enc.qexact; A.want_exact = 0; A.drop_len = 1;
+    A.raw = c->raw; A.region_cap = region_cap; A.rctr = c->rctr; A.qexact = c->enc.qexact; A.want_exact = 0; A.drop_len = 1; A.tile_rows = switches().scan_tile_rows;
     A.q_rec = c->enc.q_rec; A.e_rec = dl->e_rec;
 
     A.fuse = (switches().fuse_prefilter && switches().prefilter) ? 1 : 0;
diff --git a/include/anx.h b/include/anx.h
--- a/include/anx.h
+++ b/include/anx.h
@@ -180,6 +180,7 @@
 int anx_debug_entries(const anx_model *, uint32_t **out_vocab_ids, size_t *n);
 int anx_debug_adjacency(const anx_model *, int closure, uint64_t budget_bytes, const uint64_t *sigs, size_t n, uint32_t *out_cum,
                         uint32_t **out_ids, uint64_t *out_stats);
+int anx_debug_adj_tile_rows(const uint32_t *hdr, uint32_t k, uint32_t *out);
 int anx_debug_adjacency_device(const anx_model *, const uint64_t *sigs, size_t n, uint32_t *out_cum, uint32_t **out_ids);
 int anx_debug_band_bound(int device, const uint8_t *q_rows, const uint8_t *c_rows, const uint8_t *lq, const uint8_t *lc, size_t n,
                          int d, int form, uint8_t *out_reject);
```

After: 54.09 billion, median of 6. About the same (+0.3%).
